# mklarqvist/StormBitmaps

Hardware: AMD Instinct MI355X
Metric: 64-bit bitmap words/s, XX^T upper-tri pairwise AND+popcount (10000x65536) (higher is better)
Workload: dtype u64 (bits as exact FP4 0/1 MFMA operands, f32 accumulate < 2^24); 1 GPU; STORM_contiguous_t N=10000 M=65536 dense draws=32768 seed=42 (BASELINE configs[1], README `benchmark 65536 10000`); entry_point=storm_hip_pairw_dense_launch == STORM_contig_pairw_intersect_cardinality_blocked, kernel_variant=4, work_items=14520

## Files before the change

### stormbitmaps_amd/csrc/storm_hip.hip

```cpp
#include "storm_hip_internal.h"

#include <chrono>

#include <algorithm>
#include <atomic>
#include <cstdarg>
#include <cstdlib>
#include <cstring>

namespace storm {

static thread_local char g_error[512] = "";

void set_error(const char* fmt, ...) {
    va_list ap;
    va_start(ap, fmt);
    vsnprintf(g_error, sizeof(g_error), fmt, ap);
    va_end(ap);
}

#define STORM_PAIR(A, B)                 \
    "v_and_b32 %[t], %[" A "], %[" B "]\n\t" \
    "s_nop 0\n\t"                        \
    "v_bcnt_u32_b32 %[acc], %[t], %[acc]\n\t"
// ... 384 lines not shown
}

int storm_hip_device_pci_bus_id(int device, char* buf, size_t buflen) {
    if (!buf || buflen < 13) return STORM_HIP_EINVAL;
    STORM_HIP_TRY(hipDeviceGetPCIBusId(buf, (int)buflen, device));
    return STORM_HIP_OK;
}

namespace storm {
__global__ void warm_core_kernel() {}
}

int storm_hip_ctx_create(int device, void* stream, storm_hip_ctx_t** out) {
    if (!out) {
        set_error("storm_hip_ctx_create: NULL out");
        return STORM_HIP_EINVAL;
    }
    *out = nullptr;
    int n = 0;
    if (hipGetDeviceCount(&n) != hipSuccess || n == 0) {
        set_error("no HIP device visible (this library has no CPU fallback)");
        return STORM_HIP_ENODEV;
    }
    if (device < 0 || device >= n) {
        set_error("device %d out of range (%d visible)", device, n);
        return STORM_HIP_EINVAL;
    }
    hipDeviceProp_t prop;
    STORM_HIP_TRY(hipGetDeviceProperties(&prop, device));
    if (strncmp(prop.gcnArchName, "gfx950", 6) != 0) {
        set_error("device %d is %s; this library carries gfx950 code objects only", device,
                  prop.gcnArchName);
        return STORM_HIP_ENODEV;
    }
    STORM_HIP_TRY(hipSetDevice(device));
    storm_hip_ctx_t* ctx = new (std::nothrow) storm_hip_ctx_t();
    if (!ctx) return STORM_HIP_ENOMEM;
    ctx->device = device;
    ctx->stream = reinterpret_cast<hipStream_t>(stream);
    ctx->n_cus = prop.multiProcessorCount;
    if (hipMalloc(reinterpret_cast<void**>(&ctx->d_slots), (kSlots + kSlotsExtra) * sizeof(uint64_t)) !=
            hipSuccess ||
        hipMalloc(reinterpret_cast<void**>(&ctx->d_scalar), 64) != hipSuccess) {
        set_error("workspace allocation failed");
        storm_hip_ctx_destroy(ctx);
        return STORM_HIP_ENOMEM;
    }
    if (hipMemsetAsync(ctx->d_slots, 0, (kSlots + kSlotsExtra) * sizeof(uint64_t), ctx->stream) != hipSuccess ||
        hipMemsetAsync(ctx->d_scalar, 0, 64, ctx->stream) != hipSuccess) {
        set_error("workspace memset failed");
        storm_hip_ctx_destroy(ctx);
        return STORM_HIP_EHIP;
    }
    if (!getenv("STORM_HIP_NO_WARM")) {
        hipLaunchKernelGGL(warm_core_kernel, dim3(1), dim3(64), 0, ctx->stream);
        warm_mfma_code(ctx->stream);
        warm_sparse_code(ctx->stream);
        warm_lists_code(ctx->stream);
        (void)result_target(ctx);
        ctx->mail_armed = false;
        (void)hipStreamCreateWithFlags(&ctx->copy_stream, hipStreamNonBlocking);
        {
            std::vector<uint64_t> pageable(kSlots, 0);
            (void)hipMemcpyAsync(ctx->d_slots, pageable.data(), pageable.size() * sizeof(uint64_t), hipMemcpyHostToDevice, ctx->stream);
        }
        if (hipStreamSynchronize(ctx->stream) != hipSuccess || hipGetLastError() != hipSuccess) {
            set_error("warm-up launches failed");
            storm_hip_ctx_destroy(ctx);
            return STORM_HIP_EHIP;
        }
    }
    if (const char* v = getenv("STORM_HIP_VARIANT")) ctx->variant = atoi(v);
    if (const char* v = getenv("STORM_HIP_SEG_ROWS")) ctx->seg_rows = atoi(v);
    if (const char* v = getenv("STORM_HIP_CHUNKS_PER_ITEM")) ctx->chunks_per_item = atoi(v);
    *out = ctx;
    return STORM_HIP_OK;
}

int storm_hip_ctx_set_stream(storm_hip_ctx_t* ctx, void* stream) {
    if (check_ctx(ctx)) return STORM_HIP_EINVAL;
    hipStream_t next = reinterpret_cast<hipStream_t>(stream);
    if (next == ctx->stream) return STORM_HIP_OK;
    STORM_HIP_TRY(hipSetDevice(ctx->device));
    bool ordered = false;
    if (ctx->switch_ev || hipEventCreateWithFlags(&ctx->switch_ev, hipEventDisableTiming) == hipSuccess)
        ordered = hipEventRecord(ctx->switch_ev, ctx->stream) == hipSuccess &&
                  hipStreamWaitEvent(next, ctx->switch_ev, 0) == hipSuccess;
    if (!ordered) {
        (void)hipGetLastError();
        STORM_HIP_TRY(hipStreamSynchronize(ctx->stream));
    }
    ctx->stream = next;
    return STORM_HIP_OK;
}

int storm_hip_ctx_synchronize(storm_hip_ctx_t* ctx) {
    if (check_ctx(ctx)) return STORM_HIP_EINVAL;
    STORM_HIP_TRY(hipSetDevice(ctx->device));
    STORM_HIP_TRY(hipStreamSynchronize(ctx->stream));
    return STORM_HIP_OK;
}

int storm_hip_ctx_reserve_staging(storm_hip_ctx_t* ctx) {
    if (check_ctx(ctx)) return STORM_HIP_EINVAL;
    if (ctx->h_stage_ring) return STORM_HIP_OK;
    STORM_HIP_TRY(hipSetDevice(ctx->device));
    if (hipHostMalloc(&ctx->h_stage_ring, (size_t)24 << 20, hipHostMallocDefault) != hipSuccess) {
        ctx->h_stage_ring = nullptr;
        set_error("reserve_staging: hipHostMalloc of the 24 MiB staging ring failed");
        return STORM_HIP_ENOMEM;
    }
    return STORM_HIP_OK;
}

void storm_hip_ctx_destroy(storm_hip_ctx_t* ctx) {
    if (!ctx) return;
    (void)hipSetDevice(ctx->device);
    drain_deferred(ctx, false);
    if (ctx->d_slots) (void)hipFree(ctx->d_slots);
    if (ctx->d_scalar) (void)hipFree(ctx->d_scalar);
    ctx->d_positions.release();
    if (ctx->h_scalar) (void)hipHostFree(ctx->h_scalar);
    if (ctx->h_mail) (void)hipHostFree(ctx->h_mail);
    if (ctx->h_stage_ring) (void)hipHostFree(ctx->h_stage_ring);
    for (hipEvent_t e : ctx->stage_ev)
        if (e) (void)hipEventDestroy(e);
    if (ctx->switch_ev) (void)hipEventDestroy(ctx->switch_ev);
    ctx->segs.release();
    release_mfma_state(ctx);
    for (hipEvent_t ev : ctx->kernel_events) (void)hipEventDestroy(ev);
    delete ctx;
}

#ifdef STORM_HIP_PROBES
constexpr bool kToolsBuild = true;
#else
constexpr bool kToolsBuild = false;
#endif

struct OptionRow {
    const char* name;
    int storm_hip_ctx_s::*member;
    enum Kind { RANGE, SET, BOOL, ANY, HOOK } kind;
    int64_t lo, hi;
    int64_t step;
    std::vector<int64_t> set;
    const char* text;
    std::vector<int64_t> tools_only;
    const char* tools_text;
    int (*hook)(storm_hip_ctx_t* ctx, int64_t value);
    void (*after)(storm_hip_ctx_t* ctx, int64_t value);
};

static void drop_shadow(storm_hip_ctx_t* ctx, int64_t) { memset(ctx->x4_key, 0, sizeof(ctx->x4_key)); }
static void restart_series(storm_hip_ctx_t* ctx, int64_t value) {
    if (value == 1) ctx->kernel_events_used = 0;
}
static int set_matrix_pad(storm_hip_ctx_t* ctx, int64_t value) {
    ctx->k2_matrix_pad = value < 0 ? -1 : (int)std::min<int64_t>(value, 64);
    return STORM_HIP_OK;
}
static int set_fold_inline(storm_hip_ctx_t* ctx, int64_t value) {
    ctx->k2_fold_inline = value < 0 ? -1 : value != 0;
    return STORM_HIP_OK;
}
static int set_ring(storm_hip_ctx_t* ctx, int64_t value) {
    if (kToolsBuild ? (value < 3 || value > 5) && (value < 11 || value > 18) && value != 26 : value != 4) {
        set_error(kToolsBuild ? "k2_ring must be 3, 4 or 5 (10 + bits = timing probes)"
                              : "k2_ring: this build ships the 4-deep ring only (other depths and the timing "
                                "probes: build with STORM_HIP_PROBES, `make probes`)");
        return STORM_HIP_EINVAL;
    }
    ctx->k2_ring = (int)value;
    return STORM_HIP_OK;
}
static int set_debug(storm_hip_ctx_t* ctx, int64_t value) {
    if (kToolsBuild) {
        ctx->k2_debug = (int)value;
    } else if (value != 0) {
        set_error("k2_debug: timing probes (wrong results by design) are not in this build "
                  "(STORM_HIP_PROBES, `make probes`)");
        return STORM_HIP_EINVAL;
    }
    return STORM_HIP_OK;
}

static const std::vector<OptionRow>& option_table() {
    using C = storm_hip_ctx_s;
    constexpr auto RANGE = OptionRow::RANGE, SET = OptionRow::SET, BOOL = OptionRow::BOOL, ANY = OptionRow::ANY, HOOK = OptionRow::HOOK;
    constexpr const char* kCostText = "%s is a percentage of a full tile's time, 5..100";
    static const std::vector<OptionRow> rows = {
        {"variant", &C::variant, RANGE, -1, 5, 0, {}, "variant must be -1 (auto) or 0..5", {5},
         "variant 5 (wide 32x32x64 strips) is a form of the tools build (`make probes`), not of the shipped library"},
        {"probe_bundle", &C::probe_bundle, SET, 0, 0, 0, {-1, 1, 4},
         "probe_bundle must be -1 (auto: 1), 1 (one group of 128 rows per workgroup) or 4 (bundles of four)"},
        {"sparse_probe", &C::sparse_probe, RANGE, -1, 1, 0, {}, "sparse_probe must be -1 (auto), 0 (never) or 1 (every eligible column)"},
        {"result_mailbox", &C::result_mailbox, BOOL},
        {"sync_poll_us", &C::sync_poll_us, RANGE, 0, 1000000, 0, {}, "sync_poll_us: 0 .. 1000000 microseconds"},
        {"matrix_lists", &C::matrix_lists, RANGE, -1, 1, 0, {}, "matrix_lists must be -1 (by density), 0 (never) or 1 (whenever eligible)"},
        {"matrix_lists_kernel", &C::matrix_lists_kernel, RANGE, 0, 2, 0, {},
         "matrix_lists_kernel: 0 (by the row length), 1 (window kernel) or 2 (hash kernel)"},
        {"matrix_lists_hash_min_log2", &C::matrix_lists_hash_min_log2, RANGE, 3, 7, 0, {}, "matrix_lists_hash_min_log2: 3 .. 7"},
        {"matrix_lists_debug", &C::matrix_lists_debug, ANY},
        {"matrix_lists_density", &C::matrix_lists_permille_x10, RANGE, 0, 10000, 0, {},
         "matrix_lists_density: 0 .. 10000 (1/10000 of the dense replica's bits)"},
        {"seg_rows", &C::seg_rows, RANGE, 1, 1 << 20, 0, {}, "seg_rows out of range"},
        {"k2_stages_per_item", &C::k2_stages_per_item, RANGE, 1, 65536, 0, {}, "k2_stages_per_item out of range"},
        {"k2_max_run", &C::k2_max_run, RANGE, 0, 4096, 0, {},
         "k2_max_run out of range (0 = chosen by the list-scheduling estimate, 1..4096)"},
        {"k2_ring", &C::k2_ring, HOOK, 0, 0, 0, {}, nullptr, {}, nullptr, set_ring},
        {"k2_shadow_budget_mb", &C::k2_shadow_budget_mb, RANGE, 0, 1 << 22, 0, {}, "k2_shadow_budget_mb must be 0 (unbounded) .. 4194304",
         {}, nullptr, nullptr, drop_shadow},
        {"k2_tile_shape", &C::k2_tile_shape, SET, 0, 0, 0, {0, 1, 2, 3, 4, 5, 6, 16, 32},
         "k2_tile_shape must be 0 (chosen by the matrix), 5 (both operands as FP4 images in the LDS, 16x16x128 MFMAs), 1, 2 (bit operands inflated in registers), 3 / 4 (B as FP4 images in the LDS, 16x16x128 / 32x32x64 MFMAs), 6 (128 x 128 tiles, k-parts whose sums meet inside the launch), 16 or 32 (FP4 shadow)",
         {1, 16},
         "k2_tile_shape = 1 / 16 (tilebits_kernel, tile16_fp4_kernel) is a form of the tools build (`make probes`), not of the shipped library"},
        {"k2_ring_sync", &C::k2_ring_sync, BOOL},
        {"k2_wave_below", &C::k2_wave_below, RANGE, 0, 1 << 30, 0, {}, "k2_wave_below: 0 (never) .. 2^30 tiles of 256 x 256"},
        {"k2_part_slots", &C::k2_part_slots, RANGE, 0, 2, 0, {}, "k2_part_slots must be 0 (by the length of the segments), 1 or 2 per CU"},
        {"k2_part_min_chunks", &C::k2_part_min_chunks, RANGE, 1, 4096, 0, {}, "k2_part_min_chunks: 1 .. 4096 chunks of 512 bits"},
        {"k2_part_narrow", &C::k2_part_narrow, BOOL},
        {"k2_part_cost_diag", &C::k2_part_cost_diag, RANGE, 10, 100, 0, {}, "k2_part_cost_diag: 10 .. 100 percent of a full tile's chunk"},
        {"k2_ring_cost_diag", &C::k2_ring_cost_diag, RANGE, 5, 100, 0, {}, kCostText},
        {"k2_ring_cost_ragged", &C::k2_ring_cost_ragged, RANGE, 5, 100, 0, {}, kCostText},
        {"k2_tile_cost_diag", &C::k2_tile_cost_diag, RANGE, 5, 100, 0, {}, kCostText},
        {"k2_tile_cost_ragged", &C::k2_tile_cost_ragged, RANGE, 5, 100, 0, {}, kCostText},
        {"k2_strip_operands", &C::k2_strip_operands, RANGE, 0, 6, 0, {},
         "k2_strip_operands must be 0 (by size), 1 (bit operands, one item per workgroup), 2 (bit operands, one stream per workgroup), 3 (the same with a ring per wave), 4 (FP4 shadow), 5 (bit operands, FP4 image built in the LDS) or 6 (the same with 512-row A tiles, two halves behind one image)",
         {1, 3},
         "k2_strip_operands = 1 (stripbits_kernel) and 3 (bitwave_kernel) are forms of the tools build (`make probes`), not of the shipped library"},
        {"k2_strip_rows", &C::k2_strip_rows, SET, 0, 0, 0, {0, 64, 128},
         "k2_strip_rows must be 0 (by rule), 64 (64 A rows per wave, 256-row A tiles) or 128 (128 A rows per wave on 128-bit slices, 512-row A tiles)"},
        {"k2_shard_pairs", &C::k2_shard_pairs, BOOL},
        {"k2_matrix_pad", &C::k2_matrix_pad, HOOK, 0, 0, 0, {}, nullptr, {}, nullptr, set_matrix_pad},
        {"k2_fold_inline", &C::k2_fold_inline, HOOK, 0, 0, 0, {}, nullptr, {}, nullptr, set_fold_inline},
        {"k2_wave_ring", &C::k2_wave_ring, SET, 0, 0, 0, {0, 3, 4, 6, 8}, "k2_wave_ring must be 0 (by occupancy), 3, 4, 6 or 8"},
        {"k2_stream_max_rows", &C::k2_stream_max_rows, RANGE, 0, 1ll << 31, 0, {}, "k2_stream_max_rows must be 0 .. 2^31"},
        {"k2_stream_groups_per_cu", &C::k2_stream_groups_per_cu, RANGE, 0, 255, 0, {}, "k2_stream_groups_per_cu must be 0 (auto) .. 255"},
        {"k2_stream_min_piece", &C::k2_stream_min_piece, RANGE, 1, 4096, 0, {}, "%s must be 1..4096 stages"},
        {"k2_stream_min_run", &C::k2_stream_min_run, RANGE, 1, 4096, 0, {}, "%s must be 1..4096 stages"},
        {"k2_stream_w3_1", &C::k2_stream_w3_1, RANGE, 10, 1000, 0, {}, "%s must be 10..1000 percent of the first workgroup's share"},
        {"k2_stream_w3_2", &C::k2_stream_w3_2, RANGE, 10, 1000, 0, {}, "%s must be 10..1000 percent of the first workgroup's share"},
        {"k2_shape", &C::k2_shape, SET, 0, 0, 0, {16, 32}, "k2_shape must be 16 (16x16x128 MFMA) or 32 (32x32x64)", {32},
         "k2_shape = 32 (strip_fp4_kernel) is a form of the tools build (`make probes`), not of the shipped library"},
        {"keep_shadow", &C::keep_shadow, BOOL, 0, 0, 0, {}, nullptr, {}, nullptr, nullptr, drop_shadow},
        {"k2_matrix_parts", &C::k2_matrix_parts, BOOL},
        {"k2_matrix_min_part", &C::k2_matrix_min_part, RANGE, 4, 4096, 4, {},
         "k2_matrix_min_part: a multiple of 4 in 4 .. 4096 (stages of 128 bits)"},
        {"k2_matrix_split", &C::k2_matrix_split, BOOL},
        {"k2_pitch_pad", &C::k2_pitch_pad, RANGE, -1, 65536, 128, {}, "k2_pitch_pad must be -1 (auto) or a multiple of 128 in 0..65536"},
        {"k2_lds_pad", &C::k2_lds_pad, RANGE, 0, 120 * 1024, 0, {}, "k2_lds_pad must be 0..122880"},
        {"k2_persistent", &C::k2_persistent, BOOL, 0, 0, 0, {}, nullptr, {1},
         "k2_persistent (strip_fp4_kernel with work queues) is a form of the tools build (`make probes`), not of the shipped library"},
        {"k2_lpt_rounds", &C::k2_lpt_rounds, RANGE, 0, 63, 0, {}, "k2_lpt_rounds must be 0..63"},
        {"k2_tail_slices", &C::k2_tail_slices, RANGE, 0, 255, 0, {}, "k2_tail_slices must be 0..255"},
        {"k2_tail_run", &C::k2_tail_run, RANGE, 1, 4096, 0, {}, "k2_tail_run must be 1..4096"},
        {"k2_debug", &C::k2_debug, HOOK, 0, 0, 0, {}, nullptr, {}, nullptr, set_debug},
        {"time_kernels", &C::time_kernels, BOOL, 0, 0, 0, {}, nullptr, {}, nullptr, nullptr, restart_series},
        {"chunks_per_item", &C::chunks_per_item, RANGE, 0, 4096, 0, {}, "chunks_per_item out of range"},
    };
    return rows;
}

static const OptionRow* find_option(const char* key) {
    for (const OptionRow& row : option_table())
        if (!strcmp(key, row.name)) return &row;
    return nullptr;
}

int storm_hip_option_check(const char* key, int64_t value) {
    storm_hip_ctx_s scratch;
    scratch.n_cus = 256;
    return storm_hip_ctx_set_option(&scratch, key, value);
}

int storm_hip_ctx_set_option(storm_hip_ctx_t* ctx, const char* key, int64_t value) {
    if (check_ctx(ctx) || !key) return STORM_HIP_EINVAL;
    const OptionRow* row = find_option(key);
    if (!row) {
        set_error("unknown option '%s'", key);
        return STORM_HIP_EINVAL;
    }
    if (row->kind == OptionRow::HOOK) return row->hook(ctx, value);
    const auto among = [](const std::vector<int64_t>& set, int64_t v) { return std::find(set.begin(), set.end(), v) != set.end(); };
    const int64_t stored = row->kind == OptionRow::BOOL ? value != 0 : value;
    if ((row->kind == OptionRow::RANGE && (value < row->lo || value > row->hi || (row->step && value > 0 && value % row->step))) ||
        (row->kind == OptionRow::SET && !among(row->set, value))) {
        set_error(row->text, key);
        return STORM_HIP_EINVAL;
    }
    if (!kToolsBuild && among(row->tools_only, stored)) {
        set_error(row->tools_text, key);
        return STORM_HIP_EINVAL;
    }
    ctx->*(row->member) = (int)stored;
    if (row->after) row->after(ctx, value);
    return STORM_HIP_OK;
}

int64_t storm_hip_ctx_get_option(storm_hip_ctx_t* ctx, const char* key) {
    if (check_ctx(ctx) || !key) return -1;
    if (const OptionRow* row = find_option(key)) return ctx->*(row->member);
    if (!strcmp(key, "variant_used")) return ctx->variant_used;
    if (!strcmp(key, "k2_operands_used")) return ctx->k2_operands_used;
    if (!strcmp(key, "k2_strip_rows_used")) return ctx->k2_strip_rows_used;
    if (!strcmp(key, "k2_tile_shape_used")) return ctx->k2_tile_shape_eff;
    if (!strcmp(key, "n_cus")) return ctx->n_cus;
    if (!strcmp(key, "probes_build") || !strcmp(key, "probes_built")) return kToolsBuild;
    return -1;
}

int storm_hip_kernel_time(storm_hip_ctx_t* ctx, double* sum_ms, uint64_t* launches) {
    if (check_ctx(ctx) || !sum_ms || !launches) return STORM_HIP_EINVAL;
    STORM_HIP_TRY(hipSetDevice(ctx->device));
    STORM_HIP_TRY(hipStreamSynchronize(ctx->stream));
    *sum_ms = 0.0;
    *launches = 0;
    for (size_t i = 0; i + 1 < ctx->kernel_events_used; i += 2) {
        float ms = 0.f;
        STORM_HIP_TRY(hipEventElapsedTime(&ms, ctx->kernel_events[i], ctx->kernel_events[i + 1]));
        *sum_ms += ms;
        ++*launches;
    }
    ctx->kernel_events_used = 0;
    return STORM_HIP_OK;
}

int storm_hip_debug_strip_trace(storm_hip_ctx_t* ctx, uint64_t* out, uint64_t capacity_items,
                                uint64_t* n_items) {
    return guarded("storm_hip_debug_strip_trace", [&]() -> int {
    if (check_ctx(ctx) || !n_items) return STORM_HIP_EINVAL;
#ifndef STORM_HIP_PROBES
    set_error("strip trace: not in this build (STORM_HIP_PROBES, `make probes`)");
    *n_items = 0;
    return STORM_HIP_EINVAL;
#endif
    *n_items = ctx->trace_items;
    if (!out || ctx->trace_items == 0) return STORM_HIP_OK;
    STORM_HIP_TRY(hipSetDevice(ctx->device));
    STORM_HIP_TRY(hipStreamSynchronize(ctx->stream));
    const uint64_t n = std::min<uint64_t>(capacity_items, ctx->trace_items);
    if (ctx->trace_is_stream) {
        STORM_HIP_TRY(hipMemcpy(out, ctx->d_trace, n * 8 * sizeof(uint64_t), hipMemcpyDeviceToHost));
        return STORM_HIP_OK;
    }
    std::vector<uint64_t> raw(n * 4);
    std::vector<uint32_t> items(n * 5, 0);
    STORM_HIP_TRY(hipMemcpy(raw.data(), ctx->d_trace, n * 4 * sizeof(uint64_t), hipMemcpyDeviceToHost));
    if (!ctx->trace_is_stream)
        STORM_HIP_TRY(hipMemcpy(items.data(), ctx->strips.d, n * 5 * sizeof(uint32_t),
                                hipMemcpyDeviceToHost));
    for (uint64_t i = 0; i < n; ++i) {
        for (int k = 0; k < 4; ++k) out[i * 8 + k] = raw[i * 4 + k];
        out[i * 8 + 4] = items[i * 5 + 0];
        out[i * 8 + 5] = items[i * 5 + 1];
        out[i * 8 + 6] = (uint64_t)items[i * 5 + 3] - items[i * 5 + 2];
        out[i * 8 + 7] = items[i * 5 + 4];
    }
    return STORM_HIP_OK;
    });
}

int storm_hip_last_pass_report(storm_hip_ctx_t* ctx, uint64_t out[4]) {
    if (check_ctx(ctx) || !out) return STORM_HIP_EINVAL;
    memcpy(out, ctx->pass_report, sizeof(ctx->pass_report));
    return STORM_HIP_OK;
}

int storm_hip_last_launch_info(storm_hip_ctx_t* ctx, uint64_t out[4]) {
    if (check_ctx(ctx) || !out) return STORM_HIP_EINVAL;
    memcpy(out, ctx->last_info, sizeof(ctx->last_info));
    return STORM_HIP_OK;
}

int storm_hip_matrix_create(storm_hip_ctx_t* ctx, uint64_t n_rows, uint32_t n_words,
                            storm_hip_matrix_t** out) {
    return guarded("storm_hip_matrix_create", [&]() -> int {
    if (check_ctx(ctx) || !out) return STORM_HIP_EINVAL;
    *out = nullptr;
    if (n_words == 0 || n_rows >= (1ull << 32) - kABlockRows) {
        set_error("matrix shape out of range (rows=%llu words=%u)", (unsigned long long)n_rows,
                  n_words);
        return STORM_HIP_EINVAL;
    }
    STORM_HIP_TRY(hipSetDevice(ctx->device));
    storm_hip_matrix_t* m = new (std::nothrow) storm_hip_matrix_t();
    if (!m) return STORM_HIP_ENOMEM;
    m->n_rows = n_rows;
    m->n_words = n_words;
    m->generation = next_matrix_generation();
    m->n_rows_pad = std::max<uint64_t>(kRowPad, (n_rows + kRowPad - 1) / kRowPad * kRowPad);
    m->stride_words = ((uint64_t)n_words + kChunkWords - 1) / kChunkWords * kChunkWords;
    m->stride_words += pitch_pad_chunks(ctx->k2_matrix_pad, m->stride_words) * kChunkWords;
    const size_t bytes = m->n_rows_pad * m->stride_words * sizeof(uint64_t);
    if (hipMalloc(reinterpret_cast<void**>(&m->d), bytes) != hipSuccess) {
        set_error("hipMalloc of %zu bytes for the dense matrix failed", bytes);
        delete m;
        return STORM_HIP_ENOMEM;
    }
    if (hipMemsetAsync(m->d, 0, bytes, ctx->stream) != hipSuccess) {
        set_error("hipMemsetAsync failed");
        (void)hipFree(m->d);
        delete m;
        return STORM_HIP_EHIP;
    }
    *out = m;
    return STORM_HIP_OK;
    });
}

int storm_hip_matrix_resize(storm_hip_ctx_t* ctx, storm_hip_matrix_t* m, uint64_t n_rows) {
    return guarded("storm_hip_matrix_resize", [&]() -> int {
    if (check_ctx(ctx)) return STORM_HIP_EINVAL;
    if (!m || n_rows >= (1ull << 32) - kABlockRows) {
        set_error("matrix_resize: NULL matrix or row count out of range");
        return STORM_HIP_EINVAL;
    }
    STORM_HIP_TRY(hipSetDevice(ctx->device));
    const uint64_t row_bytes = m->stride_words * sizeof(uint64_t);
    if (n_rows > m->n_rows_pad) {
        const uint64_t want = (n_rows + kRowPad - 1) / kRowPad * kRowPad;
        const uint64_t new_pad = std::max<uint64_t>(want, 2 * m->n_rows_pad);
        uint64_t* nd = nullptr;
        if (hipMalloc(reinterpret_cast<void**>(&nd), new_pad * row_bytes) != hipSuccess) {
            set_error("matrix_resize: hipMalloc of %llu bytes failed",
                      (unsigned long long)(new_pad * row_bytes));
            return STORM_HIP_ENOMEM;
        }
        if (hipMemcpyAsync(nd, m->d, m->n_rows_pad * row_bytes, hipMemcpyDeviceToDevice,
                           ctx->stream) != hipSuccess ||
            hipMemsetAsync(nd + m->n_rows_pad * m->stride_words, 0,
                           (new_pad - m->n_rows_pad) * row_bytes, ctx->stream) != hipSuccess ||
            hipStreamSynchronize(ctx->stream) != hipSuccess) {
            (void)hipFree(nd);
            set_error("matrix_resize: device copy failed");
            return STORM_HIP_EHIP;
        }
        (void)hipFree(m->d);
        m->d = nd;
        m->n_rows_pad = new_pad;
    } else if (n_rows < m->n_rows) {
        STORM_HIP_TRY(hipMemsetAsync(m->d + n_rows * m->stride_words, 0,
                                     (m->n_rows - n_rows) * row_bytes, ctx->stream));
    }
    m->n_rows = n_rows;
    m->generation = next_matrix_generation();
    return STORM_HIP_OK;
    });
}

static int check_rows(const storm_hip_matrix_t* m, uint64_t row0, uint64_t n_rows) {
    if (!m) {
        set_error("NULL matrix");
        return STORM_HIP_EINVAL;
    }
    if (row0 + n_rows > m->n_rows || row0 + n_rows < row0) {
        set_error("rows [%llu, +%llu) outside the matrix (%llu rows)", (unsigned long long)row0,
                  (unsigned long long)n_rows, (unsigned long long)m->n_rows);
        return STORM_HIP_EINVAL;
// ... 684 lines not shown
```

### stormbitmaps_amd/csrc/storm_hip_internal.h

```cpp
#pragma once

#include <hip/hip_runtime.h>

#include <algorithm>
#include <cstdint>
#include <cstdio>
#include <exception>
#include <cstring>
#include <new>
#include <optional>
#include <thread>
#include <utility>
#include <variant>
#include <vector>

#include "storm_hip.h"
#include "storm_hip_plan.h"

struct storm_hip_ctx_s;
typedef struct storm_hip_ctx_s storm_hip_ctx_t;
struct storm_hip_matrix_s;

namespace storm {

// ... 49 lines not shown
            return STORM_HIP_ENOMEM;
        }
        capacity = bytes;
        return STORM_HIP_OK;
    }
    void release() {
        if (d) (void)hipFree(d);
        d = nullptr;
        capacity = 0;
    }
};

template <class Rec, class Key>
struct WorkList {
    DevBuf<Rec> d;
    std::optional<Key> key;
    uint32_t n = 0;
    const Rec* recs() const { return d.d; }
    bool holds(const Key& k) const { return d && key == k; }
    void forget() {
        key.reset();
        n = 0;
    }
    template <class R>
    int put(storm_hip_ctx_t* ctx, std::optional<Key>&& k, const R* recs, size_t count, const char* what, size_t floor_bytes = 0);
    void release() {
        d.release();
        forget();
    }
};

struct SegRequest {
    uint64_t n_rows;
    uint32_t shard_rank, shard_count, seg_len;
    bool operator==(const SegRequest& o) const {
        return n_rows == o.n_rows && shard_rank == o.shard_rank && shard_count == o.shard_count && seg_len == o.seg_len;
    }
};
struct SegList : WorkList<Seg, SegRequest> {
    uint64_t row_sum = 0;
};

struct ItemList : WorkList<void, std::variant<TileSumRequest, MatrixTilesRequest, Tile128Request>> {
    MatrixPlan matrix_plan;
    template <class Rq>
    bool holds(const Rq& rq) const {
        const Rq* have = key ? std::get_if<Rq>(&*key) : nullptr;
        return d && have && *have == rq;
    }
};

struct StripList : WorkList<StripItem, StripRequest> {
    uint32_t queue_base[8] = {0, 0, 0, 0, 0, 0, 0, 0};
    uint32_t queue_count[8] = {0, 0, 0, 0, 0, 0, 0, 0};
};

struct PanelList {
    WorkList<StripItem, StripRequest> list;
    hipEvent_t landed = nullptr;
};

constexpr int kLanes = 64;
constexpr int kWaves = 4;
constexpr int kThreads = kLanes * kWaves;
constexpr int kRowsPerWave = 32;
static_assert(kABlockRows == kWaves * kRowsPerWave, "128 A rows per workgroup (storm_hip_plan.h)");
constexpr int kRowPad = 256;
constexpr int kStageRows = 32;
constexpr int kSlots = 4096;
constexpr int kSlotsExtra = 8;

int launch_pairw_segments(storm_hip_ctx_t* ctx, const uint64_t* X, uint64_t stride_words,
                          const Seg* d_segs, uint32_t n_segs, uint64_t seg_row_sum,
                          uint64_t* d_total);

}

struct storm_hip_ctx_s {
    int device = 0;
    hipStream_t stream = nullptr;
    hipEvent_t switch_ev = nullptr;
    int n_cus = 0;
    unsigned long long* d_slots = nullptr;
    unsigned long long* d_scalar = nullptr;
    unsigned long long* h_scalar = nullptr;
    unsigned long long* h_mail = nullptr;
    unsigned long long* d_mail = nullptr;
    int result_mailbox = 1;
    int sync_poll_us = 0;
    bool mail_armed = false;
    std::vector<void*> deferred_free, deferred_host_free;
    uint32_t deferred_age = 0;
    hipEvent_t stage_ev[3] = {nullptr, nullptr, nullptr};
    bool stage_used[3] = {false, false, false};
    int stage_next = 0;
    void* h_stage_ring = nullptr;
    storm::SegList segs;
    int variant = -1;
    int variant_used = 2;
    int probe_bundle = -1;
    int sparse_probe = -1;
    int matrix_lists = -1;
    int matrix_lists_kernel = 0;
    int matrix_lists_hash_min_log2 = 6;
    int matrix_lists_debug = 0;
    int matrix_lists_permille_x10 = 80;
    int seg_rows = 256;
    int chunks_per_item = 0;
    uint64_t last_info[4] = {0, 0, 0, 0};
    uint64_t sparse_census[4] = {0, 0, 0, 0};
    uint64_t pass_report[4] = {0, 0, 0, 0};
    storm::DevBuf<uint8_t> d_x4;
    storm::ItemList items;
    std::vector<storm::PanelList> panel_lists;
    hipStream_t copy_stream = nullptr;
    storm::StripList strips;
    int k2_stages_per_item = 32;
    int k2_max_run = 0;
    int k2_ring = 4;
    int k2_shadow_budget_mb = 96 * 1024;
    int k2_strip_operands = 0;
    int k2_stream_max_rows = 8192;
    int k2_shard_pairs = 0;
    int k2_matrix_pad = -1;
    int k2_fold_inline = -1;
    int k2_operands_used = 4;
    int k2_strip_rows = 0;
    int k2_strip_rows_used = 64;
    int k2_tile_shape = 0;
    int k2_wave_below = 400;
    int k2_part_slots = 0;
    int k2_part_min_chunks = 8;
    int k2_part_narrow = 1;
    int k2_part_cost_diag = 80;
    storm::DevBuf<uint32_t> d_tickets;
    bool tickets_dirty = false;
    int k2_tile_shape_eff = 2;
    int k2_ring_sync = 0;
    int k2_ring_cost_diag = 78, k2_ring_cost_ragged = 40;
    int k2_tile_cost_diag = 63, k2_tile_cost_ragged = 30;
    int k2_shape = 16;
    int k2_persistent = 0;
    int keep_shadow = 0;
    uint64_t x4_key[4] = {0, 0, 0, 0};
    int k2_matrix_split = 1;
    int k2_matrix_parts = 0;
    storm::DevBuf<uint32_t> d_parts;
    int k2_matrix_min_part = 32;
    int k2_pitch_pad = -1;
    int k2_lds_pad = 0;
    int k2_lpt_rounds = 6;
    int k2_tail_slices = 3;
    int k2_tail_run = 32;
    int time_kernels = 0;
    std::vector<hipEvent_t> kernel_events;
    size_t kernel_events_used = 0;
    storm::DevBuf<uint32_t> d_band;
    storm::DevBuf<uint64_t> d_dosage_rows;
    storm::DevBuf<uint32_t> d_dosage_sums;
    storm::DevBuf<void> d_positions;
    storm::DevBuf<uint32_t> d_counts;
    storm::DevBuf<unsigned long long> d_trace;
    uint32_t trace_items = 0;
    storm::WorkList<uint32_t, storm::BitstreamRequest> bitfirst;
    storm::DevBuf<storm::BitSeg> d_bitsegs;
    uint32_t n_bit_groups = 0, n_bit_segs = 0, bit_max_stages = 0;
    uint64_t bit_stages = 0;
    int k2_stream_groups_per_cu = 0;
    int k2_stream_min_piece = 6;
    int k2_stream_min_run = 2;
    int k2_stream_w3_1 = 120, k2_stream_w3_2 = 60;
    int k2_wave_ring = 0;
    bool trace_is_stream = false;
    int k2_debug = 0;
};

namespace storm {
int launch_pairw_mfma(storm_hip_ctx_t* ctx, const storm_hip_matrix_s* m, uint32_t shard_rank,
                      uint32_t shard_count, uint64_t* d_total);
int launch_pairw_mfma_ranges(storm_hip_ctx_t* ctx, const uint64_t* X, uint64_t stride_words,
                             uint64_t n_rows_src, uint64_t n_rows_dst,
                             const std::vector<RowRange>& ranges, uint32_t shard_rank,
                             uint32_t shard_count, int strip_mode, uint64_t* d_total,
                             uint64_t shadow_generation = 0, uint32_t n_words_logical = 0);
int launch_pairw_bits_upload(storm_hip_ctx_t* ctx, storm_hip_matrix_s* m, const uint64_t* host_rows,
                             uint64_t src_stride_words, uint64_t* d_total);
int stage_check_lists(const storm_hip_stage_s* stage, const std::vector<uint64_t>& ltable);
int stage_gather_lists(storm_hip_ctx_t* ctx, storm_hip_stage_s* stage, const std::vector<uint64_t>& ltable, uint16_t* d_lists,
                       uint64_t** d_table);
int strip_operands_of(const storm_hip_ctx_t* ctx);
int launch_pairw_bits_ranges(storm_hip_ctx_t* ctx, const uint8_t* X, uint64_t pitch_bytes,
                             const std::vector<RowRange>& ranges, uint32_t n_kslices2, uint32_t shard_rank,
                             uint32_t shard_count, uint64_t* d_total, bool slots_hold_sums = false,
                             uint32_t a_tile = 256u,
                             bool rows128 = false);
static inline uint64_t ranges_word_pairs(const std::vector<RowRange>& ranges, uint64_t words, uint32_t shard_count) {
    uint64_t pairs = 0;
    for (const RowRange& rg : ranges) {
        const uint64_t n = rg.r1 - rg.r0, a = rg.a_end ? std::min(rg.a_end, rg.r1) - rg.r0 : n;
        pairs += a * (a - (a != 0)) / 2 + a * (n - a);
    }
    return pairs * words / (shard_count ? shard_count : 1);
}
int launch_pairw_matrix(storm_hip_ctx_t* ctx, const storm_hip_matrix_s* m, int op, uint32_t* d_out,
                        uint64_t ld, uint64_t band_row0 = 0, uint64_t band_rows = ~0ull);
int launch_pairw_lag_matrix(storm_hip_ctx_t* ctx, const storm_hip_matrix_s* m, int op, uint64_t max_lag, uint64_t band_row0,
                            uint64_t band_rows, uint32_t* d_out, uint64_t ld);
int launch_pairw_dosage_matrix(storm_hip_ctx_t* ctx, const storm_hip_matrix_s* m, uint32_t* d_out, uint64_t ld);
int launch_pairw_lag_dosage_matrix(storm_hip_ctx_t* ctx, const storm_hip_matrix_s* m, uint64_t max_lag, uint64_t band_row0,
                                   uint64_t band_rows, uint32_t* d_out, uint64_t ld);
int launch_square_dosage_matrix(storm_hip_ctx_t* ctx, const storm_hip_matrix_s* a, const storm_hip_matrix_s* b, uint32_t* d_out,
                                uint64_t ld);
int launch_square_mfma(storm_hip_ctx_t* ctx, const storm_hip_matrix_s* a,
                       const storm_hip_matrix_s* b, uint64_t* d_total);
int launch_square_matrix(storm_hip_ctx_t* ctx, const storm_hip_matrix_s* a,
                         const storm_hip_matrix_s* b, int op, uint32_t* d_out, uint64_t ld);
int launch_row_counts(storm_hip_ctx_t* ctx, const storm_hip_matrix_s* m, uint32_t* d_counts);
int launch_similarity_finish(storm_hip_ctx_t* ctx, void* d_io, uint64_t ld, uint64_t n_rows, uint64_t n_cols,
                             const uint32_t* d_counts_rows, const uint32_t* d_counts_cols, int triangle, int measure,
                             uint64_t n_bits);
int launch_similarity_finish_lag(storm_hip_ctx_t* ctx, void* d_io, uint64_t ld, uint64_t n_rows, uint64_t row0,
                                 uint64_t n_band_rows, uint64_t max_lag, const uint32_t* d_counts, int measure, uint64_t n_bits);
int launch_lag_band_sums(storm_hip_ctx_t* ctx, const float* d_vals, uint64_t ld, uint64_t n_rows, uint64_t max_lag, int stat,
                         uint64_t n_const, const uint32_t* d_nobs, uint64_t nobs_row_pitch, uint64_t nobs_col_stride,
                         float* d_score, uint32_t* d_n_pairs);
constexpr uint32_t kLdscoreMaxAnnot = 1024;
int launch_lag_band_annot_sums(storm_hip_ctx_t* ctx, const float* d_vals, uint64_t ld, uint64_t n_rows, uint64_t max_lag, int stat,
                               uint64_t n_const, const uint32_t* d_nobs, uint64_t nobs_row_pitch, uint64_t nobs_col_stride,
                               const uint32_t* d_lo, const uint32_t* d_hi, const float* d_annot, uint64_t annot_ld,
                               uint64_t n_annot, float* d_score, uint64_t score_ld, uint32_t* d_n_pairs);
int check_lag_band_prune(const char* who, uint64_t n_rows, const uint32_t* h_lo, const uint32_t* h_hi, float min_r2);
size_t lag_band_prune_scratch_words(uint64_t n_rows, uint64_t lag, bool windows, bool order);
int launch_lag_band_prune(storm_hip_ctx_t* ctx, const char* who, const float* d_vals, uint64_t ld, uint64_t n_rows, uint64_t lag,
                          float min_r2, const uint32_t* h_lo, const uint32_t* h_hi, const uint32_t* h_order, uint8_t* d_keep,
                          uint32_t* d_owner, uint32_t* d_scratch);
void release_mfma_state(storm_hip_ctx_t* ctx);
void drain_deferred(storm_hip_ctx_t* ctx, bool aged);
void warm_mfma_code(hipStream_t stream);
void warm_sparse_code(hipStream_t stream);
void warm_lists_code(hipStream_t stream);
int fetch_result_word(storm_hip_ctx_t* ctx, uint64_t* h_total);
uint64_t* result_target(storm_hip_ctx_t* ctx);
int wait_mailbox(storm_hip_ctx_t* ctx, uint64_t* value);
int launch_fold_slots(storm_hip_ctx_t* ctx, uint64_t* d_total);
void kernel_time_mark(storm_hip_ctx_t* ctx);
uint64_t next_matrix_generation();
struct Piece { const void* src; size_t bytes; size_t dst_off; size_t zero_after = 0; };
struct Stager {
    static constexpr size_t kBuf = 8u << 20;
    static constexpr int kBufs = 3;
    storm_hip_ctx_t* ctx;
    hipEvent_t (&ev)[kBufs];
    bool (&used)[kBufs];
    int& next;
    explicit Stager(storm_hip_ctx_t* c) : ctx(c), ev(c->stage_ev), used(c->stage_used), next(c->stage_next) {}
    static_assert(kBuf * kBufs == ((size_t)24 << 20), "storm_hip_ctx_reserve_staging allocates the same ring");
    int init() {
        if (!ctx->h_stage_ring) {
            if (hipHostMalloc(&ctx->h_stage_ring, kBuf * kBufs, hipHostMallocDefault) != hipSuccess) {
                ctx->h_stage_ring = nullptr;
                set_error("sparse_create: hipHostMalloc of the %zu-byte staging ring failed", kBuf * kBufs);
                return STORM_HIP_ENOMEM;
            }
        }
        for (int i = 0; i < kBufs; ++i)
            if (!ev[i] && hipEventCreateWithFlags(&ev[i], hipEventDisableTiming) != hipSuccess) return STORM_HIP_EHIP;
        return STORM_HIP_OK;
    }
    int send(uint8_t* d_base, const Piece* pieces, size_t n, size_t span) {
        uint8_t* buf = static_cast<uint8_t*>(ctx->h_stage_ring) + (size_t)next * kBuf;
        if (used[next] && hipEventSynchronize(ev[next]) != hipSuccess) return STORM_HIP_EHIP;
        const unsigned parts = span >= (1u << 20) ? 4u : 1u;
        auto pack = [&](unsigned part) {
            for (size_t i = n * part / parts; i < n * (part + 1) / parts; ++i) {
                memcpy(buf + pieces[i].dst_off, pieces[i].src, pieces[i].bytes);
                if (pieces[i].zero_after) memset(buf + pieces[i].dst_off + pieces[i].bytes, 0, pieces[i].zero_after);
            }
        };
        if (parts > 1) {
            std::thread helpers[3];
            for (unsigned t = 1; t < parts; ++t) helpers[t - 1] = std::thread(pack, t);
            pack(0);
            for (unsigned t = 1; t < parts; ++t) helpers[t - 1].join();
        } else {
            pack(0);
        }
        if (hipMemcpyAsync(d_base, buf, span, hipMemcpyHostToDevice, ctx->stream) != hipSuccess ||
            hipEventRecord(ev[next], ctx->stream) != hipSuccess)
            return STORM_HIP_EHIP;
        used[next] = true;
        next = (next + 1) % kBufs;
        return STORM_HIP_OK;
    }
    int send_rows(uint8_t* d_base, const std::vector<const void*>& rows, size_t bytes, size_t stride) {
        const size_t per_chunk = kBuf / stride;
        std::vector<Piece> chunk;
        for (size_t r0 = 0; r0 < rows.size(); r0 += per_chunk) {
            const size_t n = std::min(per_chunk, rows.size() - r0);
            chunk.clear();
            for (size_t i = 0; i < n; ++i) chunk.push_back({rows[r0 + i], bytes, i * stride, stride - bytes});
            if (int rc = send(d_base + r0 * stride, chunk.data(), n, n * stride)) return rc;
        }
        return STORM_HIP_OK;
    }
    int send_run(uint8_t* d_base, const std::vector<std::pair<const void*, size_t>>& run) {
        std::vector<Piece> chunk;
// ... 115 lines not shown
```

### stormbitmaps_amd/csrc/storm_hip_mfma.hip

```cpp
#include "storm_hip_internal.h"

#include <algorithm>
#include <chrono>
#include <cstring>
#include <exception>
#include <type_traits>
#include <utility>

namespace storm {

#ifdef STORM_HIP_PROBES
__device__ unsigned long long g_clock_probe[4];
#define STORM_CLOCK_BEGIN()                                  \
    const uint64_t ck_t0 = __builtin_amdgcn_s_memtime();     \
    const uint64_t ck_r0 = __builtin_amdgcn_s_memrealtime()
#define STORM_CLOCK_END()                                                                           \
    do {                                                                                            \
        if (threadIdx.x == 0) {                                                                     \
            atomicAdd(&g_clock_probe[0], (unsigned long long)(__builtin_amdgcn_s_memtime() - ck_t0)); \
            atomicAdd(&g_clock_probe[1], (unsigned long long)(__builtin_amdgcn_s_memrealtime() - ck_r0)); \
            atomicAdd(&g_clock_probe[2], 1ull);                                                     \
        }                                                                                           \
    } while (0)
#else
// ... 1010 lines not shown
            STORM_BS_FETCH(x1, t, 1, 0);
            STORM_BS_FETCH(x2, t, 0, 1);
            STORM_BS_FETCH(x3, t, 1, 1);
            asm volatile("s_waitcnt lgkmcnt(0)" : "+v"(x1), "+v"(x2), "+v"(x3)::"memory");
            __builtin_amdgcn_sched_barrier(0);
            a[0][0][0] = tb_inflate<0>(w0); a[0][1][0] = tb_inflate<1>(w0);
            a[0][2][0] = tb_inflate<2>(w0); a[0][3][0] = tb_inflate<3>(w0);
            a[0][0][1] = tb_inflate<0>(x1); a[0][1][1] = tb_inflate<1>(x1);
            a[0][2][1] = tb_inflate<2>(x1); a[0][3][1] = tb_inflate<3>(x1);
            a[1][0][0] = tb_inflate<0>(x2); a[1][1][0] = tb_inflate<1>(x2);
            a[1][2][0] = tb_inflate<2>(x2); a[1][3][0] = tb_inflate<3>(x2);
            a[1][0][1] = tb_inflate<0>(x3); a[1][1][1] = tb_inflate<1>(x3);
            a[1][2][1] = tb_inflate<2>(x3); a[1][3][1] = tb_inflate<3>(x3);
            if (diag) {
#pragma unroll
                for (int k = 0; k < 4; ++k)
                    dbits += __builtin_popcount((uint32_t)w0[k]) + __builtin_popcount((uint32_t)x1[k]) +
                             __builtin_popcount((uint32_t)x2[k]) + __builtin_popcount((uint32_t)x3[k]);
            }
        }
        if (mul) {
            const int half = (own && ci < 4u) ? 1 : 0;
            sb[0] = tb_scale<0>() - half;
            sb[1] = tb_scale<1>() - half;
            sb[2] = tb_scale<2>() - half;
            sb[3] = tb_scale<3>() - half;
            __builtin_amdgcn_sched_barrier(0);
            STORM_BS_STAGE(t, tn);
            STORM_BS_WAIT();
            STORM_BS_KEEP();
        } else {
            STORM_BS_FETCH(w0, tn, 0, 0);
            asm volatile("s_waitcnt lgkmcnt(0)" : "+v"(w0)::"memory");
            __builtin_amdgcn_sched_barrier(0);
            e0 = tb_inflate<0>(w0);
        }
        if (kTrace) {
            const unsigned long long now = __builtin_readcyclecounter();
            c_body += now - c_mark;
            c_mark = now;
            n_mul += mul ? 1u : 0u;
        }
        if (kTrace) c_issue += __builtin_readcyclecounter() - c_mark;
        ++t;
        ++ci;
        if (ci == 4u + rc.n_b) {
            ci = 0;
            ++sc;
            rc = segs[min(sc, s_end - 1u)];
        }
    }
#undef STORM_BS_STAGE
#undef STORM_BS_KEEP
#undef STORM_BS_WAIT
#undef STORM_BS_STEP
#undef STORM_BS_FETCH

    long long mine2 = 0;
#pragma unroll
    for (int m = 0; m < 2; ++m) {
        uint32_t part = 0;
#pragma unroll
        for (int n = 0; n < 2; ++n)
#pragma unroll
            for (int r = 0; r < 16; ++r) part += (uint32_t)(acc[m][n][r] * 2.0f);
        mine2 += part;
    }
    mine2 -= (long long)dbits;
#pragma unroll
    for (int o = 32; o > 0; o >>= 1) mine2 += __shfl_down(mine2, o, 64);
    __builtin_amdgcn_s_barrier();
    long long* wsum = reinterpret_cast<long long*>(lds_raw);
    if (lane == 0) wsum[wave] = mine2;
    __syncthreads();
    if (tid == 0) {
        const long long tot2 = wsum[0] + wsum[1] + wsum[2] + wsum[3];
        if (tot2 != 0) atomicAdd(&slots[blockIdx.x & (kBsFoldSlots - 1)], (unsigned long long)(tot2 / 2));
        __threadfence();
        const unsigned long long arrived = atomicAdd(&slots[kBsTicket], 1ull);
        wsum[4] = (arrived == (unsigned long long)gridDim.x - 1ull) ? 1 : 0;
        if (kTrace) {
            trace[blockIdx.x * 8ull + 0] = t_start;
            trace[blockIdx.x * 8ull + 1] = __builtin_amdgcn_s_memrealtime();
            trace[blockIdx.x * 8ull + 2] = ((t_ready - t_start) & 0xffffffffull) | ((unsigned long long)t << 32);
            trace[blockIdx.x * 8ull + 3] = __builtin_amdgcn_s_getreg(20 | (0 << 6) | (31 << 11)) |
                                           ((unsigned long long)__builtin_amdgcn_s_getreg(4 | (0 << 6) | (31 << 11)) << 32);
            trace[blockIdx.x * 8ull + 4] = c_wait;
            trace[blockIdx.x * 8ull + 5] = c_issue;
            trace[blockIdx.x * 8ull + 6] = c_body;
            trace[blockIdx.x * 8ull + 7] = n_mul;
        }
    }
    __syncthreads();
    if (wsum[4] != 0 && wave == 0) {
        __threadfence();
        unsigned long long v = __hip_atomic_exchange(&slots[lane], 0ull, __ATOMIC_RELAXED, __HIP_MEMORY_SCOPE_AGENT);
#pragma unroll
        for (int o = 32; o > 0; o >>= 1) v += __shfl_down(v, o, 64);
        if (lane == 0) {
            out[0] = v;
            __hip_atomic_store(&slots[kBsTicket], 0ull, __ATOMIC_RELAXED, __HIP_MEMORY_SCOPE_AGENT);
        }
    }
}

#ifdef STORM_HIP_PROBES
#include "../../tools/probes/bitwave.hip"
#endif

static void release_panel_lists(storm_hip_ctx_t* ctx) {
    for (PanelList& l : ctx->panel_lists) {
        l.list.release();
        if (l.landed) (void)hipEventDestroy(l.landed);
    }
    ctx->panel_lists.clear();
    if (ctx->copy_stream) (void)hipStreamDestroy(ctx->copy_stream);
    ctx->copy_stream = nullptr;
}

__global__ void warm_mfma_kernel() {}
void warm_mfma_code(hipStream_t stream) { hipLaunchKernelGGL(warm_mfma_kernel, dim3(1), dim3(64), 0, stream); }

void release_mfma_state(storm_hip_ctx_t* ctx) {
    release_panel_lists(ctx);
    ctx->d_x4.release();
    ctx->items.release();
    ctx->strips.release();
    ctx->d_trace.release();
    ctx->d_counts.release();
    ctx->d_band.release();
    ctx->d_dosage_rows.release();
    ctx->d_dosage_sums.release();
    ctx->d_parts.release();
    ctx->d_tickets.release();
    ctx->d_bitsegs.release();
    ctx->bitfirst.release();
}

constexpr size_t kItemsFloorBytes = 4096 * sizeof(MfmaItem);
constexpr size_t kStripItemsFloorBytes = 4096 * sizeof(StripItem);

static int ensure_items(storm_hip_ctx_t* ctx, const std::vector<RowRange>& ranges,
                        uint32_t total_stages, uint32_t shard_rank, uint32_t shard_count,
                        bool diag_only) {
    const TileSumRequest rq = {ranges_hash(ranges), total_stages, shard_rank, shard_count,
                               (uint32_t)std::max(1, ctx->k2_stages_per_item), diag_only ? 1u : 0u,
                               (ctx->k2_debug & 3) == 1 ? 1u : 0u};
    if (ctx->items.holds(rq)) return STORM_HIP_OK;
    std::vector<MfmaItem> items;
    if (int rc = plan_tile_sum(rq, ranges, items)) return rc;
    return ctx->items.put(ctx, rq, items.data(), items.size(), "K2: the item table", kItemsFloorBytes);
}

static StripOptions strip_options_of(const storm_hip_ctx_t* ctx, int xcd_group) {
    StripOptions o;
    o.max_run = ctx->k2_max_run;
    o.tail_run = ctx->k2_tail_run;
    o.tail_slices = ctx->k2_tail_slices;
    o.lpt_rounds = ctx->k2_lpt_rounds;
    o.shard_pairs = ctx->k2_shard_pairs != 0;
    o.n_cus = ctx->n_cus;
    o.xcd_group = xcd_group;
    o.persistent = ctx->k2_persistent != 0;
    o.one_slice_probe = (ctx->k2_debug & 16) != 0;
    return o;
}

static int ensure_strip_items(storm_hip_ctx_t* ctx, const std::vector<RowRange>& ranges,
                              uint32_t n_kslices, uint32_t shard_rank, uint32_t shard_count,
                              uint32_t a_tile, int xcd_group = 1) {
    const StripRequest rq = strip_request(strip_options_of(ctx, xcd_group), ranges, n_kslices, shard_rank, shard_count, a_tile);
    if (ctx->strips.holds(rq)) return STORM_HIP_OK;
    ctx->strips.forget();
    std::vector<StripItem> items;
    plan_strips(rq, ranges, items, ctx->strips.queue_base, ctx->strips.queue_count);
    if (items.size() >= (1ull << 31)) {
        set_error("K2s: %zu strip items exceed the grid limit", items.size());
        return STORM_HIP_EINVAL;
    }
    return ctx->strips.put(ctx, rq, items.data(), items.size(), "K2s: the strip items", kStripItemsFloorBytes);
}

static uint64_t shadow_pitch(const storm_hip_ctx_t* ctx, uint64_t row_bytes) {
    if (ctx->k2_pitch_pad >= 0) return row_bytes + (uint64_t)ctx->k2_pitch_pad;
    return row_bytes + (row_bytes % 1024 == 0 ? 384u : 0u);
}
static int ensure_shadow(storm_hip_ctx_t* ctx, size_t bytes, const char* what) {
    if (bytes > ctx->d_x4.capacity) memset(ctx->x4_key, 0, sizeof(ctx->x4_key));
    return ctx->d_x4.ensure(bytes, what);
}

int launch_pairw_mfma_ranges(storm_hip_ctx_t* ctx, const uint64_t* X, uint64_t stride_words,
                             uint64_t n_rows_src, uint64_t n_rows_dst,
                             const std::vector<RowRange>& ranges, uint32_t shard_rank,
                             uint32_t shard_count, int strip_mode, uint64_t* d_total,
                             uint64_t shadow_generation, uint32_t n_words_logical) {
    const bool strips = strip_mode != 0;
    const uint32_t a_tile = strip_mode == 2 ? 512u : (uint32_t)kStripATile;
    const uint64_t row_bytes = stride_words * 32;
    const uint32_t n_kslices = n_words_logical
                                   ? (n_words_logical + 3u) / 4u
                                   : (uint32_t)(row_bytes / kStripRowBytes);
    const uint64_t rows_alloc = std::max<uint64_t>(n_rows_dst, kTile);
    uint32_t n_chunks = 1, chunk_slices = n_kslices;
    uint64_t shadow_row_bytes = row_bytes;
    if (strips) {
        uint64_t want = 1;
        if (ctx->k2_shadow_budget_mb > 0) {
            const uint64_t budget = (uint64_t)ctx->k2_shadow_budget_mb << 20;
            const uint64_t full = rows_alloc * shadow_pitch(ctx, row_bytes);
            if (full > budget && n_kslices > 8) want = (full + budget - 1) / budget;
        }
        constexpr uint32_t kDmaCapSlices = ((1u << 26) - 1024u) / kStripRowBytes / 8u * 8u;
        want = std::max<uint64_t>(want, ((uint64_t)n_kslices + kDmaCapSlices - 1) / kDmaCapSlices);
        if (want > 1) {
            chunk_slices = (uint32_t)(((uint64_t)n_kslices + want - 1) / want + 7u) / 8u * 8u;
            chunk_slices = std::min(chunk_slices, kDmaCapSlices);
            n_chunks = (n_kslices + chunk_slices - 1) / chunk_slices;
            shadow_row_bytes = (uint64_t)chunk_slices * kStripRowBytes;
        }
    }
    const uint64_t pitch = shadow_pitch(ctx, shadow_row_bytes);
    const size_t x4_bytes = (size_t)rows_alloc * pitch;
    if (n_rows_dst / kTile >= 65535) {
        set_error("K2: too many row blocks");
        return STORM_HIP_EINVAL;
    }
    if (int rc = ensure_shadow(ctx, x4_bytes, "K2: the FP4 shadow matrix")) return rc;
    const uint32_t total_stages = (uint32_t)(row_bytes / kStageBytes);
    if (strips) {
        ctx->items.forget();
    } else if (int rc = ensure_items(ctx, ranges, total_stages, shard_rank, shard_count, false)) {
        return rc;
    }
    if (pitch * (uint64_t)(strips ? kStripBRows : kTile) >= (1ull << 32)) {
        set_error("K2: rows of %llu nibble bytes exceed the 32-bit DMA offsets; use variant 2",
                  (unsigned long long)shadow_row_bytes);
        return STORM_HIP_EINVAL;
    }
    if (strips)
        if (int rc = ensure_strip_items(ctx, ranges, chunk_slices, shard_rank, shard_count, a_tile))
            return rc;
    if ((uint64_t)ctx->k2_stages_per_item * 128u >= (1u << 24)) {
        set_error("K2: k-slice too long for exact f32 accumulation");
        return STORM_HIP_EINVAL;
    }
    const uint32_t n_strip = strips ? ctx->strips.n : 0;
    const uint32_t n_tiles = ctx->items.n;
    const uint64_t key[4] = {(uint64_t)(uintptr_t)X, shadow_generation,
                             ((uint64_t)shard_rank << 32) | shard_count,
                             (pitch << 20) ^ (n_rows_dst << 2) ^ (uint64_t)strip_mode};
    const bool shadow_valid = ctx->keep_shadow && shadow_generation != 0 && n_chunks == 1 &&
                              !memcmp(key, ctx->x4_key, sizeof(key)) &&
                              (ctx->k2_debug >> 8) == 0;
    const ExpandOwn own = strips ? ExpandOwn{shard_rank, shard_count, 5u,
                                             ctx->k2_shard_pairs ? 0u
                                                                 : strip_modulo_slices(chunk_slices, shard_count) / kOwnSlices}
                                 : ExpandOwn{shard_rank, shard_count, 7u, 0xffffffffu};
    const uint32_t nib = (ctx->k2_debug >> 8) ? (uint32_t)(ctx->k2_debug >> 8) & 15u : 2u;
    const uint64_t n_src = std::min(n_rows_src, n_rows_dst);
    for (uint32_t chunk = 0; chunk < n_chunks && (n_tiles > 0 || n_strip > 0); ++chunk) {
        if (!shadow_valid) {
            if (n_chunks == 1) {
                hipLaunchKernelGGL(expand_fp4_kernel,
                                   expand_grid(n_rows_dst, stride_words, expand_compact_halves(own, stride_words * 2)),
                                   dim3(256), 0, ctx->stream, X, stride_words, n_src, n_rows_dst,
                                   reinterpret_cast<uint4*>(ctx->d_x4.d), own, nib, pitch / 16);
            } else {
                const uint64_t h0 = (uint64_t)chunk * chunk_slices * 8u, h1 = h0 + (uint64_t)chunk_slices * 8u;
                hipLaunchKernelGGL(expand_fp4_kernel,
                                   expand_grid(n_rows_dst, stride_words, expand_compact_halves(own, h1 - h0)),
                                   dim3(256), 0, ctx->stream, X, stride_words, n_src, n_rows_dst,
                                   reinterpret_cast<uint4*>(ctx->d_x4.d), own, nib, pitch / 16, h0, h1, h0);
            }
        }
        STORM_HIP_TRY(hipGetLastError());
        if (n_chunks == 1) memcpy(ctx->x4_key, key, sizeof(key));
        else memset(ctx->x4_key, 0, sizeof(ctx->x4_key));
        if (n_strip > 0) {
            kernel_time_mark(ctx);
            const StripItem* sit = ctx->strips.d;
            const dim3 sgrid(n_strip), sblock(kStripThreads);
#ifdef STORM_HIP_PROBES
            StripQueues queues;
            memcpy(queues.base, ctx->strips.queue_base, sizeof(queues.base));
            memcpy(queues.count, ctx->strips.queue_count, sizeof(queues.count));
            unsigned int* heads = reinterpret_cast<unsigned int*>(ctx->d_slots + kSlots);
            const dim3 pgrid(std::min<uint32_t>(n_strip, (uint32_t)ctx->n_cus * (strip_mode == 2 ? 2u : 4u)));
            const bool persist = ctx->k2_persistent && n_chunks == 1;
            const int sel = strip_mode == 2 ? 100 + ctx->k2_ring
                                            : (persist && ctx->k2_ring == 4) ? 204
                                            : (persist && ctx->k2_ring == 18) ? 218
                                                                              : ctx->k2_ring;
            switch (sel) {
#include "../../tools/probes/strip_fp4_32_launch.hip"
                default:
                    if (ctx->k2_shape != 16)
                        hipLaunchKernelGGL(strip_fp4_kernel<kStripRingDefault>, sgrid, sblock,
                                           (size_t)ctx->k2_lds_pad, ctx->stream, ctx->d_x4, pitch, sit,
                                           ctx->d_slots);
                    else
                        hipLaunchKernelGGL(strip16_fp4_kernel<kStripRingDefault>, sgrid, sblock,
                                           (size_t)ctx->k2_lds_pad, ctx->stream, ctx->d_x4, pitch, sit,
                                           ctx->d_slots);
                    break;
            }
#else
            hipLaunchKernelGGL(strip16_fp4_kernel<kStripRingDefault>, sgrid, sblock, (size_t)ctx->k2_lds_pad, ctx->stream,
                               ctx->d_x4, pitch, sit, ctx->d_slots);
#endif
            kernel_time_mark(ctx);
            STORM_HIP_TRY(hipGetLastError());
        }
        if (n_tiles > 0) {
            kernel_time_mark(ctx);
            const dim3 kgrid(n_tiles), block(kMfmaThreads);
            const MfmaItem* items = static_cast<const MfmaItem*>(ctx->items.recs());
            switch (ctx->k2_debug & 12) {
#ifdef STORM_HIP_PROBES
                case 4:
                    hipLaunchKernelGGL(pairw_fp4_kernel<4>, kgrid, block, 0, ctx->stream, ctx->d_x4,
                                       pitch, items, ctx->d_slots);
                    break;
                case 8:
                    hipLaunchKernelGGL(pairw_fp4_kernel<8>, kgrid, block, 0, ctx->stream, ctx->d_x4,
                                       pitch, items, ctx->d_slots);
                    break;
#endif
// ... 392 lines not shown
int launch_square_matrix(storm_hip_ctx_t* ctx, const storm_hip_matrix_s* a,
                         const storm_hip_matrix_s* b, int op, uint32_t* d_out, uint64_t ld) {
    if (a->n_rows == 0 || b->n_rows == 0) return STORM_HIP_OK;
    ctx->k2_tile_shape_eff = (ctx->k2_tile_shape && ctx->k2_tile_shape != 6) ? ctx->k2_tile_shape : ((a->sparse_origin && b->sparse_origin) ? 2 : 5);
    const uint64_t stride_words = a->stride_words;
    const uint64_t row_bytes = stride_words * 32;
    const bool bits = ctx->k2_tile_shape_eff <= 5 && b->stride_words == stride_words;
    const uint64_t pitch = bits ? stride_words * 8 : shadow_pitch(ctx, row_bytes);
    const uint64_t rows_a = (a->n_rows + kTile - 1) / kTile * kTile;
    const uint64_t rows_b = (b->n_rows + kTile - 1) / kTile * kTile;
    if (int rc = check_tile_limits("square_matrix", pitch, kTile, (rows_a + rows_b) / kTile + 1, false)) return rc;
    const size_t x4_bytes = bits ? 0 : (size_t)(rows_a + rows_b) * pitch;
    if (int rc = ensure_shadow(ctx, x4_bytes, "square_matrix: the FP4 shadow")) return rc;
    const uint32_t total_stages = bits ? (std::max(a->n_words, b->n_words) + 7u) / 8u * 4u : (uint32_t)(row_bytes / kStageBytes);
    const uint32_t ta = (uint32_t)(rows_a / kTile), tb = (uint32_t)(rows_b / kTile);
    const bool k2h = choose_tile128(ctx, (uint64_t)ta * tb, pitch, bits);
    int rc = STORM_HIP_OK;
    MatrixPlan plan;
    if (k2h) {
        ctx->k2_tile_shape_eff = 6;
    } else {
        MatrixTilesRequest rq;
        rq.total_stages = total_stages;
        xcd_grouped_tiles(0, ta, ta, ta + tb, false, rq.tiles);
        rc = ensure_matrix_tiles(ctx, std::move(rq), &plan);
    }
    uint32_t* d_counts = nullptr;
    if (rc == STORM_HIP_OK) rc = op_row_counts(ctx, op, a, b, rows_a, rows_a + rows_b, &d_counts);
    if (rc == STORM_HIP_OK) {
        const OutWindow w = rectangle_window(d_out, ld, a->n_rows, rows_a, b->n_rows, d_counts, op);
        for (int side = 0; side < 2 && !bits; ++side) {
            const storm_hip_matrix_s* m = side ? b : a;
            const uint64_t rows_dst = side ? rows_b : rows_a;
            const dim3 grid = expand_grid(rows_dst, stride_words);
            hipLaunchKernelGGL(expand_fp4_kernel, grid, dim3(256), 0, ctx->stream, m->d,
                               stride_words, std::min<uint64_t>(m->n_rows_pad, rows_dst), rows_dst,
                               reinterpret_cast<uint4*>(ctx->d_x4.d + (side ? rows_a * pitch : 0)),
                               kExpandAll, 2u, pitch / 16);
        }
        const TileOperands ops = bits ? operands_of(a->d, b->d, pitch, rows_a, std::min<uint64_t>(a->n_rows_pad, rows_a),
                                                    std::min<uint64_t>(b->n_rows_pad, rows_b))
                                      : operands_of(ctx->d_x4.d, pitch, rows_a + rows_b);
        rc = k2h ? run_tile128(ctx, total_stages, ops, w, 1u) : run_matrix_tiles(ctx, plan, ops, bits, w);
    }
    if (rc == STORM_HIP_EHIP) set_error("square_matrix: HIP failure");
    return rc;
}

static BitstreamRequest bitstream_request_of(const storm_hip_ctx_t* ctx, const std::vector<RowRange>& ranges, uint32_t n_kslices,
                                             uint32_t shard_rank, uint32_t shard_count, uint64_t pitch) {
    BitstreamShaping sh;
    sh.groups_per_cu = ctx->k2_stream_groups_per_cu;
    sh.min_piece = std::max(1, ctx->k2_stream_min_piece);
    sh.min_run = std::max(1, ctx->k2_stream_min_run);
    sh.w3_1 = ctx->k2_stream_w3_1;
    sh.w3_2 = ctx->k2_stream_w3_2;
    return bitstream_request(sh, ranges, n_kslices, shard_rank, shard_count, (uint32_t)std::max(1, ctx->n_cus), pitch);
}

static int ensure_bitstream(storm_hip_ctx_t* ctx, const std::vector<RowRange>& ranges, uint32_t n_kslices,
                            uint32_t shard_rank, uint32_t shard_count, uint64_t pitch) {
    const BitstreamRequest rq = bitstream_request_of(ctx, ranges, n_kslices, shard_rank, shard_count, pitch);
    if (ctx->bitfirst.holds(rq)) return STORM_HIP_OK;
    ctx->bitfirst.forget();
    BitstreamPlan plan;
    build_bitstream(rq, ranges, plan);
    if (plan.bases.size() >= (1ull << 32) ||
        (!ranges.empty() && ranges.back().r1 * pitch / 64 + n_kslices >= (1ull << 32))) {
        set_error("K2q: the matrix is beyond the 32-bit stage addresses (64-byte units)");
        return STORM_HIP_EINVAL;
    }
    if (plan.max_stages > kBsMaxStages) {
        set_error("K2q: a workgroup of %u stages exceeds the exact range of its accumulators", plan.max_stages);
        return STORM_HIP_EINVAL;
    }
    const size_t seg_bytes = std::max<size_t>(plan.segs.size(), 1) * sizeof(BitSeg);
    std::vector<uint32_t> packed(plan.first);
    packed.insert(packed.end(), plan.first_stage.begin(), plan.first_stage.end());
    packed.insert(packed.end(), plan.bases.begin(), plan.bases.end());
    packed.push_back(0u);
    if (int rc = ctx->d_bitsegs.ensure(seg_bytes, "K2q: the segment table")) return rc;
    if (upload_bytes(ctx, ctx->d_bitsegs, plan.segs.data(), plan.segs.size() * sizeof(BitSeg))) {
        set_error("K2q: the segment table: the copy to the device failed");
        return STORM_HIP_EHIP;
    }
    ctx->n_bit_groups = plan.groups;
    ctx->bit_stages = plan.stages;
    ctx->bit_max_stages = plan.max_stages;
    ctx->n_bit_segs = (uint32_t)plan.segs.size();
    return ctx->bitfirst.put(ctx, rq, packed.data(), packed.size(), "K2q: the workgroups' stage tables");
}

int launch_pairw_bitstream(storm_hip_ctx_t* ctx, const uint64_t* X, uint64_t pitch,
                           const std::vector<RowRange>& ranges, uint32_t n_kslices, uint32_t shard_rank,
                           uint32_t shard_count, uint64_t* d_total) {
    if (pitch * (uint64_t)kStripBRows >= (1ull << 32) || pitch % 64 != 0) {
        set_error("K2q: rows of %llu bytes are outside the bit-operand stream's 32-bit DMA offsets",
                  (unsigned long long)pitch);
        return STORM_HIP_EINVAL;
    }
    if (int rc = ensure_bitstream(ctx, ranges, n_kslices, shard_rank, shard_count, pitch)) return rc;
    ctx->pass_report[0] |= STORM_HIP_RAN_BITSTREAM;
    ctx->pass_report[1] += ranges_word_pairs(ranges, (uint64_t)n_kslices * 8u, shard_count);
    ctx->items.forget();
    ctx->last_info[0] = ctx->n_bit_groups;
    ctx->last_info[1] = ctx->bit_max_stages;
    ctx->last_info[2] = 1;
    ctx->last_info[3] = ctx->n_bit_segs;
    if (ctx->n_bit_groups == 0)
        return launch_fold_slots(ctx, d_total);
    kernel_time_mark(ctx);
    const dim3 grid(ctx->n_bit_groups), block(kStripThreads);
#ifdef STORM_HIP_PROBES
    if (ctx->k2_ring == 18) {
        const size_t need = (size_t)ctx->n_bit_groups * 8 * sizeof(unsigned long long);
        if (int rc = ctx->d_trace.ensure(need, "K2q: the schedule trace")) return rc;
        ctx->trace_items = ctx->n_bit_groups;
        ctx->trace_is_stream = true;
        hipLaunchKernelGGL(bitstream_kernel<true>, grid, block, 0, ctx->stream,
                           reinterpret_cast<const uint8_t*>(X), pitch, ctx->d_bitsegs.d,
                           ctx->bitfirst.recs(),
                           ctx->bitfirst.recs() + 2 * ((size_t)ctx->n_bit_groups + 1),
                           ctx->bitfirst.recs() + ((size_t)ctx->n_bit_groups + 1), ctx->d_slots,
                           reinterpret_cast<unsigned long long*>(d_total), ctx->d_trace);
    } else
#endif
        hipLaunchKernelGGL(bitstream_kernel<false>, grid, block, 0, ctx->stream,
                           reinterpret_cast<const uint8_t*>(X), pitch, ctx->d_bitsegs.d,
                           ctx->bitfirst.recs(),
                           ctx->bitfirst.recs() + 2 * ((size_t)ctx->n_bit_groups + 1),
                           ctx->bitfirst.recs() + ((size_t)ctx->n_bit_groups + 1), ctx->d_slots,
                           reinterpret_cast<unsigned long long*>(d_total), (unsigned long long*)nullptr);
    kernel_time_mark(ctx);
    STORM_HIP_TRY(hipGetLastError());
    return STORM_HIP_OK;
}

#ifdef STORM_HIP_PROBES
#include "../../tools/probes/bitwave_launch.hip"
#endif

int launch_pairw_bits_ranges(storm_hip_ctx_t* ctx, const uint8_t* X, uint64_t pitch,
                             const std::vector<RowRange>& ranges, uint32_t n_kslices2, uint32_t shard_rank,
                             uint32_t shard_count, uint64_t* d_total, bool slots_hold_sums, uint32_t a_tile, bool rows128) {
    if (pitch * (uint64_t)kStripBRows >= (1ull << 32)) {
        set_error("K2b: rows of %llu bytes are beyond the strips' 32-bit DMA offsets", (unsigned long long)pitch);
        return STORM_HIP_EINVAL;
    }
    ctx->items.forget();
    if (rows128 && a_tile != kStripRowsATile) {
        set_error("K2b: the 128-rows-per-wave form takes A tiles of 512 rows");
        return STORM_HIP_EINVAL;
    }
    if (int rc = ensure_strip_items(ctx, ranges, n_kslices2, shard_rank, shard_count, a_tile, rows128 ? (int)kStripRowsXcdGroup : 2))
        return rc;
    const uint32_t n_strip = ctx->strips.n;
    const uint32_t waves = rows128 ? 4u : a_tile / (uint32_t)kStripBRows;
    ctx->k2_operands_used = waves == 8u ? 6 : 5;
    ctx->k2_strip_rows_used = rows128 ? 128 : 64;
    if (n_strip > 0) {
        ctx->pass_report[0] |= STORM_HIP_RAN_BIT_STRIPS;
        ctx->pass_report[1] += ranges_word_pairs(ranges, (uint64_t)n_kslices2 * (rows128 ? 2u : 4u), shard_count);
    }
    ctx->last_info[0] = n_strip;
    ctx->last_info[1] = ctx->k2_stages_per_item;
    ctx->last_info[2] = 1;
    ctx->last_info[3] = 0;
    const uint32_t fold_slots = n_strip <= 4096u ? 256u : (uint32_t)kSlots;
    const bool fold_wanted = ctx->k2_fold_inline > 0 || (ctx->k2_fold_inline < 0 && n_strip <= 4096u);
    const uint64_t arrivals_per_slot = (uint64_t)n_strip * (uint64_t)waves / (uint64_t)fold_slots + 1u;
    const uint64_t wave_sum_max = rows128 ? 128ull * (4096ull * 64ull + 512ull) * 128ull
                                          : 64ull * (4096ull * 64ull + 256ull) * 256ull;
    const bool fold_inline = fold_wanted && !slots_hold_sums && n_strip > 0 && arrivals_per_slot < 65535u &&
                             arrivals_per_slot * wave_sum_max < (1ull << 48);
    if (n_strip > 0) {
        kernel_time_mark(ctx);
        if (rows128) {
            const bool plain = ranges.size() == 1 && ranges[0].r0 == 0 && ranges[0].a_end == 0 && ranges[0].back_from == ~0ull &&
                               ranges[0].r1 < (uint64_t)kStripRowsNoTrim;
            hipLaunchKernelGGL(strip16_rows_kernel, dim3(n_strip), dim3(256), (size_t)ctx->k2_lds_pad,
                               ctx->stream, X, pitch, ctx->strips.recs(), ctx->d_slots,
                               fold_inline ? reinterpret_cast<unsigned long long*>(d_total) : nullptr, fold_slots,
                               plain ? (uint32_t)ranges[0].r1 : kStripRowsNoTrim);
        } else if (waves == 8u)
            hipLaunchKernelGGL(strip16_bits2_kernel, dim3(n_strip), dim3(512), (size_t)ctx->k2_lds_pad,
                               ctx->stream, X, pitch, ctx->strips.recs(), ctx->d_slots,
                               fold_inline ? reinterpret_cast<unsigned long long*>(d_total) : nullptr, fold_slots);
        else
            hipLaunchKernelGGL(strip16_bits_kernel, dim3(n_strip), dim3(kStripThreads), (size_t)ctx->k2_lds_pad,
                               ctx->stream, X, pitch, ctx->strips.recs(), ctx->d_slots,
                               fold_inline ? reinterpret_cast<unsigned long long*>(d_total) : nullptr, fold_slots);
        kernel_time_mark(ctx);
        STORM_HIP_TRY(hipGetLastError());
    }
    return fold_inline ? STORM_HIP_OK : launch_fold_slots(ctx, d_total);
}

static bool strip_rows128_by_rule(const storm_hip_matrix_s* m, uint32_t shard_count) {
    return shard_count == 1 && m->n_rows >= 2048 && m->n_words >= 1024;
}
static bool strip_rows128(const storm_hip_ctx_t* ctx, const storm_hip_matrix_s* m, uint32_t shard_count) {
    if (ctx->k2_strip_rows == 64 || ctx->k2_strip_operands == 6 || (m->n_rows + kStripRowsATile - 1) / kStripRowsATile * kStripRowsATile > m->n_rows_pad) return false;
    return ctx->k2_strip_rows == 128 || strip_rows128_by_rule(m, shard_count);
}

static int launch_pairw_bits(storm_hip_ctx_t* ctx, const storm_hip_matrix_s* m, uint32_t shard_rank,
                             uint32_t shard_count, int operands, uint64_t* d_total) {
    const uint64_t pitch = m->stride_words * 8;
    const uint64_t n_rows4 = (m->n_rows + kStripATile - 1) / kStripATile * kStripATile;
    if (n_rows4 > m->n_rows_pad || pitch * (uint64_t)kStripBRows >= (1ull << 32)) {
        set_error("K2sb: matrix of %llu rows (%llu allocated) x %llu bytes per row is outside the bit-operand strips' reach",
                  (unsigned long long)m->n_rows, (unsigned long long)m->n_rows_pad, (unsigned long long)pitch);
        return STORM_HIP_EINVAL;
    }
    std::vector<RowRange> ranges;
    if (m->n_rows > 1) ranges.push_back({0, m->n_rows});
    const uint32_t n_kslices = (m->n_words + 7u) / 8u;
    if (operands == 2)
        return launch_pairw_bitstream(ctx, m->d, pitch, ranges, n_kslices, shard_rank, shard_count, d_total);
#ifdef STORM_HIP_PROBES
    if (operands == 3)
        return launch_pairw_bitwave(ctx, m->d, pitch, ranges, n_kslices, shard_rank, shard_count, d_total);
#endif
    ctx->items.forget();
    if (operands == 5 && strip_rows128(ctx, m, shard_count))
        return launch_pairw_bits_ranges(ctx, reinterpret_cast<const uint8_t*>(m->d), pitch, ranges, strip_rows_kslices(m->n_words),
                                        shard_rank, shard_count, d_total, false, kStripRowsATile, true);
    if (operands == 5 || operands == 6)
        return launch_pairw_bits_ranges(ctx, reinterpret_cast<const uint8_t*>(m->d), pitch, ranges, n_kslices * 2u,
                                        shard_rank, shard_count, d_total, false, operands == 6 ? 512u : (uint32_t)kStripATile, false);
    if (int rc = ensure_strip_items(ctx, ranges, n_kslices, shard_rank, shard_count, (uint32_t)kStripATile))
        return rc;
#ifndef STORM_HIP_PROBES
    set_error("k2_strip_operands = 1 (stripbits_kernel) is in the tools build only (`make probes`)");
    return STORM_HIP_EINVAL;
#else
    const uint32_t n_strip = ctx->strips.n;
    if (n_strip > 0) {
        kernel_time_mark(ctx);
        hipLaunchKernelGGL(stripbits_kernel, dim3(n_strip), dim3(kStripThreads), 0, ctx->stream,
                           reinterpret_cast<const uint8_t*>(m->d), pitch,
                           ctx->strips.recs(), ctx->d_slots);
        kernel_time_mark(ctx);
        STORM_HIP_TRY(hipGetLastError());
    }
    ctx->last_info[0] = n_strip;
    ctx->last_info[1] = ctx->k2_stages_per_item;
    ctx->last_info[2] = 1;
    ctx->last_info[3] = 0;
    return launch_fold_slots(ctx, d_total);
#endif
}

static int pairw_bits_upload_queue(storm_hip_ctx_t* ctx, storm_hip_matrix_s* m, const uint64_t* host_rows,
                                   uint64_t src_stride_words, uint64_t* d_total);
int launch_pairw_bits_upload(storm_hip_ctx_t* ctx, storm_hip_matrix_s* m, const uint64_t* host_rows,
                             uint64_t src_stride_words, uint64_t* d_total) {
    const int rc = pairw_bits_upload_queue(ctx, m, host_rows, src_stride_words, d_total);
    if (rc != STORM_HIP_OK) {
        if (ctx->copy_stream) (void)hipStreamSynchronize(ctx->copy_stream);
        (void)hipStreamSynchronize(ctx->stream);
        ctx->mail_armed = false;
    }
    return rc;
}
static int pairw_bits_upload_queue(storm_hip_ctx_t* ctx, storm_hip_matrix_s* m, const uint64_t* host_rows,
                                   uint64_t src_stride_words, uint64_t* d_total) {
    const uint64_t pitch = m->stride_words * 8;
    const uint64_t tiles = (m->n_rows + kStripATile - 1) / kStripATile;
    if (tiles * kStripATile > m->n_rows_pad || pitch * (uint64_t)kStripBRows >= (1ull << 32) || m->n_rows < 2) {
        set_error("pairw_dense_upload: matrix outside the bit-operand strips' reach");
        return STORM_HIP_EINVAL;
    }
    if (!ctx->copy_stream) STORM_HIP_TRY(hipStreamCreateWithFlags(&ctx->copy_stream, hipStreamNonBlocking));
    std::vector<PanelList>& lists = ctx->panel_lists;
    if (lists.empty()) lists.resize(1);
    if (!lists[0].landed) STORM_HIP_TRY(hipEventCreateWithFlags(&lists[0].landed, hipEventDisableTiming));
    STORM_HIP_TRY(hipEventRecord(lists[0].landed, ctx->stream));
    STORM_HIP_TRY(hipStreamWaitEvent(ctx->copy_stream, lists[0].landed, 0));
    std::vector<uint64_t> first_tile;
    {
        const uint64_t n = std::max<uint64_t>(1, std::min<uint64_t>(8, tiles / 4));
        for (uint64_t p = 0; p <= n; ++p) first_tile.push_back(tiles * p / n);
    }
    const uint64_t n_panels = first_tile.size() - 1;
    const uint32_t n_kslices2 = 2u * ((m->n_words + 7u) / 8u);
    if (lists.size() < n_panels) lists.resize(n_panels);
    ctx->pass_report[0] |= STORM_HIP_RAN_BIT_STRIPS;
    ctx->pass_report[1] += ranges_word_pairs({{0, m->n_rows}}, (uint64_t)n_kslices2 * 4u, 1);
    ctx->k2_operands_used = 5;
    ctx->k2_strip_rows_used = 64;
    uint64_t n_total = 0;
    for (uint64_t p = 0; p < n_panels; ++p) {
        const uint64_t t0 = first_tile[p], t1 = first_tile[p + 1];
        if (t0 >= t1) continue;
        const uint64_t row0 = t0 * kStripATile, row1 = std::min<uint64_t>(m->n_rows, t1 * kStripATile);
        PanelList& l = lists[p];
        if (!l.landed) STORM_HIP_TRY(hipEventCreateWithFlags(&l.landed, hipEventDisableTiming));
        STORM_HIP_TRY(hipMemcpy2DAsync(m->d + row0 * m->stride_words, pitch, host_rows + row0 * src_stride_words,
                                       src_stride_words * 8, (size_t)m->n_words * 8, row1 - row0, hipMemcpyHostToDevice,
                                       ctx->copy_stream));
        STORM_HIP_TRY(hipEventRecord(l.landed, ctx->copy_stream));
        StripOptions po = strip_options_of(ctx, 2);
        po.max_run = 128;
        po.shard_pairs = po.persistent = po.one_slice_probe = 0;
        RowRange rg{0, row1};
        rg.back_from = row0;
        const std::vector<RowRange> panel = {rg};
        const StripRequest rq = strip_request(po, panel, n_kslices2, 0, 1, (uint32_t)kStripATile);
        if (!l.list.holds(rq)) {
            std::vector<StripItem> items;
            uint32_t qb[8], qc[8];
            plan_strips(rq, panel, items, qb, qc);
            if (items.size() >= (1ull << 31)) {
                set_error("pairw_dense_upload: %zu strip items exceed the grid limit", items.size());
                return STORM_HIP_EINVAL;
            }
            if (int rc = l.list.put(ctx, rq, items.data(), items.size(), "pairw_dense_upload: a panel's strip items", 1024 * sizeof(StripItem)))
                return rc;
        }
        STORM_HIP_TRY(hipStreamWaitEvent(ctx->stream, l.landed, 0));
        if (l.list.n) {
            hipLaunchKernelGGL(strip16_bits_kernel, dim3(l.list.n), dim3(kStripThreads), (size_t)ctx->k2_lds_pad, ctx->stream,
                               reinterpret_cast<const uint8_t*>(m->d), pitch, l.list.recs(), ctx->d_slots,
                               (unsigned long long*)nullptr, (uint32_t)kSlots);
            STORM_HIP_TRY(hipGetLastError());
        }
        n_total += l.list.n;
    }
    ctx->last_info[0] = n_total;
    ctx->last_info[1] = ctx->k2_stages_per_item;
    ctx->last_info[2] = 1;
    ctx->last_info[3] = n_panels;
    return launch_fold_slots(ctx, d_total);
}

int strip_operands_of(const storm_hip_ctx_t* ctx) {
    if (ctx->k2_strip_operands == 6) return 5;
    if (ctx->k2_strip_operands != 0) return ctx->k2_strip_operands;
    return (ctx->k2_ring == kStripRingDefault && ctx->k2_shape == 16) ? 5 : 4;
}
int launch_pairw_mfma(storm_hip_ctx_t* ctx, const storm_hip_matrix_s* m, uint32_t shard_rank,
                      uint32_t shard_count, uint64_t* d_total) {
    const int strip_mode = ctx->variant == 5 ? 2 : ctx->variant == 4 ? 1 : 0;
    const int operands = strip_operands_of(ctx);
    if (strip_mode == 1 && (operands == 1 || operands == 2 || operands == 3 || operands == 5) && !ctx->k2_persistent && ctx->k2_debug == 0 &&
        (m->n_rows + kStripATile - 1) / kStripATile * kStripATile <= m->n_rows_pad &&
        m->stride_words * 8 * (uint64_t)kStripBRows < (1ull << 32))
    {
        const bool wide = operands == 5 && ctx->k2_strip_operands == 6 && (m->n_rows + 511u) / 512u * 512u <= m->n_rows_pad;
        ctx->k2_operands_used = wide ? 6 : operands;
        return launch_pairw_bits(ctx, m, shard_rank, shard_count, wide ? 6 : operands, d_total);
    }
    ctx->k2_operands_used = 4;
    const uint64_t tile = strip_mode == 2 ? 512 : kStripATile;
    const uint64_t n_rows4 = (m->n_rows + tile - 1) / tile * tile;
    std::vector<RowRange> ranges;
    if (m->n_rows > 1) ranges.push_back({0, m->n_rows});
    return launch_pairw_mfma_ranges(ctx, m->d, m->stride_words, m->n_rows_pad, n_rows4, ranges,
                                    shard_rank, shard_count, strip_mode, d_total, m->generation,
                                    m->n_words);
}

}

#ifdef STORM_HIP_PROBES
extern "C" int storm_hip_probe_clock(uint64_t out[3]) {
    unsigned long long v[4] = {0, 0, 0, 0};
    if (hipDeviceSynchronize() != hipSuccess) return STORM_HIP_EINVAL;
    if (hipMemcpyFromSymbol(v, HIP_SYMBOL(storm::g_clock_probe), sizeof(v)) != hipSuccess) return STORM_HIP_EINVAL;
    out[0] = v[0];
    out[1] = v[1];
    out[2] = v[2];
    const unsigned long long z[4] = {0, 0, 0, 0};
    if (hipMemcpyToSymbol(HIP_SYMBOL(storm::g_clock_probe), z, sizeof(z)) != hipSuccess) return STORM_HIP_EINVAL;
    return STORM_HIP_OK;
}
#endif
```

### stormbitmaps_amd/csrc/storm_hip_plan.cpp

```cpp
#include "storm_hip_plan.h"

#include <algorithm>
#include <cmath>
#include <cstdio>
#include <cstdlib>
#include <chrono>
#include <exception>

#include "storm_hip.h"

namespace storm {

bool timing_env() {
    static const bool on = getenv("STORM_HIP_TIMING") != nullptr;
    return on;
}

uint64_t ranges_hash(const std::vector<RowRange>& ranges) {
    uint64_t h = 1469598103934665603ull;
    for (const RowRange& r : ranges) {
        h = (h ^ r.r0) * 1099511628211ull;
        h = (h ^ r.r1) * 1099511628211ull;
        h = (h ^ r.a_end) * 1099511628211ull;
        h = (h ^ r.back_from) * 1099511628211ull;
    }
    return h;
}

int plan_tile_sum(const TileSumRequest& rq, const std::vector<RowRange>& ranges, std::vector<MfmaItem>& items) {
    const uint32_t total_stages = rq.total_stages, shard_rank = rq.shard_rank, shard_count = rq.shard_count;
    const uint32_t spi = std::max(1u, rq.stages_per_item);
    const bool diag_only = rq.diag_only != 0;
    std::vector<std::pair<uint16_t, uint16_t>> tiles;
    for (const RowRange& rg : ranges) {
        const uint32_t b0 = (uint32_t)(rg.r0 / kTile);
        const uint32_t nT = (uint32_t)((rg.r1 - rg.r0 + kTile - 1) / kTile);
        const uint32_t nTa = rg.a_end ? (uint32_t)std::min<uint64_t>(nT, (std::min(rg.a_end, rg.r1) - rg.r0 + kTile - 1) / kTile) : nT;
        for (uint32_t gi = 0; gi < nTa; gi += 4)
            for (uint32_t gj = gi / 8 * 8; gj < nT; gj += 8)
                for (uint32_t i = gi; i < std::min(gi + 4, nTa); ++i)
                    for (uint32_t j = std::max(gj, i); j < std::min(gj + 8, nT); ++j)
                        if (!diag_only || i == j)
                            tiles.emplace_back((uint16_t)(b0 + i), (uint16_t)(b0 + j));
    }
    std::vector<std::pair<uint32_t, uint32_t>> slices;
    for (uint32_t g0 = 0; g0 < total_stages; g0 += kGroupStages) {
        if ((g0 / kGroupStages) % shard_count != shard_rank) continue;
        const uint32_t g1 = std::min(total_stages, g0 + kGroupStages);
        for (uint32_t s0 = g0; s0 < g1; s0 += spi) slices.emplace_back(s0, std::min(spi, g1 - s0));
    }
    items.clear();
    const size_t n = tiles.size();
    for (const auto& sl : slices) {
        const uint32_t s0 = sl.first, ns = sl.second;
        for (size_t c = 0; c < n; c += 256)
            for (size_t pos = 0; pos < 32; ++pos)
                for (size_t x = 0; x < 8; ++x) {
                    const size_t L = c + x * 32 + pos;
                    if (L >= n) continue;
                    if (rq.one_tile_probe)
                        items.push_back({tiles[0].first, tiles[0].first, s0, ns});
                    else
                        items.push_back({tiles[L].first, tiles[L].second, s0, ns});
                }
    }
    if (items.size() != slices.size() * n) {
        set_error("K2 item table construction lost tiles (%zu != %zu)", items.size(),
                  slices.size() * n);
        return STORM_HIP_EINVAL;
    }
    if (items.size() >= (1ull << 31)) {
        set_error("K2: %zu tile items exceed the grid limit", items.size());
        return STORM_HIP_EINVAL;
    }
    return STORM_HIP_OK;
}

static inline uint32_t strip_item_cost(const StripItem& it, uint32_t per_tile) {
    return (it.j1 - it.j0) + it.diag * per_tile + 10u;
}

struct StripShaping {
    int max_run = 128, tail_run = 32, tail_slices = 3, lpt_rounds = 6;
    int xcd_group = 1;
    bool persistent = false, one_slice_probe = false;
    bool pair_space = false;
};
static void build_strip_items(const StripShaping& sh, const std::vector<RowRange>& ranges,
                              uint32_t n_kslices, uint32_t shard_rank, uint32_t shard_count,
                              uint32_t a_tile, std::vector<StripItem>& items,
                              uint32_t queue_base[8], uint32_t queue_count[8], double* makespan = nullptr,
                              uint32_t slots_per_xcd = 128) {
    const uint32_t kMaxRun = (uint32_t)std::min(4096, std::max(1, sh.max_run));
    const uint32_t kTailRun = (uint32_t)std::min(4096, std::max(1, sh.tail_run));
    const uint32_t kPerTile = a_tile / kStripBRows;
    std::vector<std::vector<uint32_t>> slices_of(8);
    uint32_t local = 0;
    const bool pair_mode = sh.pair_space && shard_count > 1;
    const uint32_t modulo_slices = pair_mode ? n_kslices : strip_modulo_slices(n_kslices, shard_count);
    const uint32_t xg = (uint32_t)std::max(1, sh.xcd_group);
    for (uint32_t ks = 0; ks < modulo_slices; ++ks)
        if (pair_mode || strip_owns_slice(ks, shard_rank, shard_count)) slices_of[(local++ / xg) % 8].push_back(ks);
    std::vector<uint64_t> pair_load(shard_count, 0);
    auto emit_slice_all = [&](uint32_t ks, uint32_t max_run, std::vector<StripItem>& dst) {
        const uint32_t ks_data = sh.one_slice_probe ? ks % 8u : ks;
        for (const RowRange& rg : ranges) {
            if (rg.back_from != ~0ull) {
                const uint32_t blk0 = (uint32_t)(rg.r0 / kStripBRows);
                for (uint64_t a0 = rg.back_from; a0 < rg.r1; a0 += a_tile) {
                    const uint32_t a_row0 = (uint32_t)a0, end = (uint32_t)(a0 / kStripBRows);
                    if (end <= blk0) {
                        dst.push_back({a_row0, 1, end, end, ks_data});
                        continue;
                    }
                    for (uint32_t j0 = blk0; j0 < end; j0 += max_run)
                        dst.push_back({a_row0, (uint32_t)(j0 == blk0), j0, std::min(end, j0 + max_run), ks_data});
                }
                continue;
            }
            const uint64_t a_rows = (rg.a_end ? std::min(rg.a_end, rg.r1) : rg.r1) - rg.r0;
            const uint32_t nA = (uint32_t)((a_rows + a_tile - 1) / a_tile);
            const uint32_t jend = (uint32_t)((rg.r1 + kStripBRows - 1) / kStripBRows);
            for (uint32_t i = 0; i < nA; ++i) {
                const uint32_t a_row0 = (uint32_t)rg.r0 + i * a_tile;
                const uint32_t first = a_row0 / (uint32_t)kStripBRows + kPerTile;
                if (first >= jend) {
                    dst.push_back({a_row0, 1, first, first, ks_data});
                    continue;
                }
                for (uint32_t j0 = first; j0 < jend; j0 += max_run)
                    dst.push_back({a_row0, (uint32_t)(j0 == first), j0,
                                   std::min(jend, j0 + max_run), ks_data});
            }
        }
    };
    const uint32_t kTailLen = std::min(kMaxRun, kTailRun);
    std::vector<StripItem> proto_main, proto_tail;
    bool have_main = false, have_tail = false;
    auto by_length = [&](const StripItem& p, const StripItem& q) {
        return (p.j1 - p.j0) + p.diag * kPerTile > (q.j1 - q.j0) + q.diag * kPerTile;
    };
    auto emit_copy = [&](uint32_t ks, uint32_t max_run, std::vector<StripItem>& dst) {
        std::vector<StripItem>& proto = max_run == kMaxRun ? proto_main : proto_tail;
        bool& have = max_run == kMaxRun ? have_main : have_tail;
        if (!have) {
            emit_slice_all(0u, max_run, proto);
            if (max_run == kMaxRun) std::stable_sort(proto.begin(), proto.end(), by_length);
            have = true;
        }
        const uint32_t ks_data = sh.one_slice_probe ? ks % 8u : ks;
        const size_t at = dst.size();
        dst.insert(dst.end(), proto.begin(), proto.end());
        for (size_t k = at; k < dst.size(); ++k) dst[k].ks = ks_data;
    };
    auto emit_slice = [&](uint32_t ks, uint32_t max_run, std::vector<StripItem>& dst) {
        if (!pair_mode) return (max_run == kMaxRun || max_run == kTailLen) ? emit_copy(ks, max_run, dst) : emit_slice_all(ks, max_run, dst);
        std::vector<StripItem> all;
        emit_slice_all(ks, max_run, all);
        std::stable_sort(all.begin(), all.end(), [&](const StripItem& p, const StripItem& q) {
            return strip_item_cost(p, kPerTile) > strip_item_cost(q, kPerTile);
        });
        for (const StripItem& it : all) {
            const uint32_t r = (uint32_t)(std::min_element(pair_load.begin(), pair_load.end()) - pair_load.begin());
            pair_load[r] += strip_item_cost(it, kPerTile);
            if (r == shard_rank) dst.push_back(it);
        }
    };
    std::vector<std::vector<StripItem>> leftover_of(8);
    if (modulo_slices < n_kslices) {
        std::vector<uint64_t> load(shard_count, 0);
        for (uint32_t ks = modulo_slices; ks < n_kslices; ++ks) {
            std::vector<StripItem> all;
            emit_slice_all(ks, std::min(kMaxRun, kTailRun), all);
            std::stable_sort(all.begin(), all.end(), [&](const StripItem& p, const StripItem& q) {
                return strip_item_cost(p, kPerTile) > strip_item_cost(q, kPerTile);
            });
            const uint32_t xcd = (local++ / xg) % 8;
            for (const StripItem& it : all) {
                const uint32_t r = (uint32_t)(std::min_element(load.begin(), load.end()) - load.begin());
                load[r] += strip_item_cost(it, kPerTile);
                if (r == shard_rank) leftover_of[xcd].push_back(it);
            }
        }
    }
    const uint32_t kTail = (uint32_t)std::max(0, sh.tail_slices);
    std::vector<std::vector<StripItem>> per_xcd(8);
    const int n_lists = makespan ? 1 : 8;
    for (int x = 0; x < n_lists; ++x) {
        const std::vector<uint32_t>& sl = slices_of[x];
        const size_t n_main = sl.size() > kTail ? sl.size() - kTail : 0;
        for (size_t k = 0; k < n_main; ++k) {
            if (!pair_mode) {
                emit_slice(sl[k], kMaxRun, per_xcd[x]);
                continue;
            }
            std::vector<StripItem> one;
            emit_slice(sl[k], kMaxRun, one);
            std::stable_sort(one.begin(), one.end(), by_length);
            per_xcd[x].insert(per_xcd[x].end(), one.begin(), one.end());
        }
        std::vector<StripItem> tail;
        for (size_t k = n_main; k < sl.size(); ++k) emit_slice(sl[k], std::min(kMaxRun, kTailRun), tail);
        tail.insert(tail.end(), leftover_of[x].begin(), leftover_of[x].end());
        std::stable_sort(tail.begin(), tail.end(), [&](const StripItem& p, const StripItem& q) {
            return (p.j1 - p.j0) + p.diag * kPerTile > (q.j1 - q.j0) + q.diag * kPerTile;
        });
        per_xcd[x].insert(per_xcd[x].end(), tail.begin(), tail.end());
        if (per_xcd[x].size() <= (size_t)128 * (size_t)std::max(0, sh.lpt_rounds))
            std::stable_sort(per_xcd[x].begin(), per_xcd[x].end(),
                             [&](const StripItem& p, const StripItem& q) {
                                 return (p.j1 - p.j0) + p.diag * kPerTile > (q.j1 - q.j0) + q.diag * kPerTile;
                             });
    }
    if (makespan) {
        auto cost_of = [&](const StripItem& it) { return (double)(it.j1 - it.j0) + (it.diag ? kPerTile + 3.0 : 0.0) + 5.0; };
        const std::vector<StripItem>& list = per_xcd[0];
        const size_t n_slots = std::max<uint32_t>(1, slots_per_xcd);
        const size_t start = list.size() > 16 * n_slots ? list.size() - 16 * n_slots : 0;
        double before = 0;
        for (size_t k = 0; k < start; ++k) before += cost_of(list[k]);
        std::vector<double> slot(n_slots, before / (double)n_slots);
        auto later = [](double p, double q) { return p > q; };
        for (size_t k = start; k < list.size(); ++k) {
            std::pop_heap(slot.begin(), slot.end(), later);
            slot.back() += cost_of(list[k]);
            std::push_heap(slot.begin(), slot.end(), later);
        }
        const double worst = *std::max_element(slot.begin(), slot.end());
        *makespan = worst;
        items.clear();
        return;
    }
    items.clear();
    if (sh.persistent) {
        for (int x = 0; x < 8; ++x) {
            queue_base[x] = (uint32_t)items.size();
            queue_count[x] = (uint32_t)per_xcd[x].size();
            items.insert(items.end(), per_xcd[x].begin(), per_xcd[x].end());
        }
    } else {
        size_t longest = 0;
        for (auto& v : per_xcd) longest = std::max(longest, v.size());
        for (size_t pos = 0; pos < longest; ++pos)
            for (int x = 0; x < 8; ++x)
                if (pos < per_xcd[x].size()) items.push_back(per_xcd[x][pos]);
    }
}

static StripShaping choose_strip_shaping(const StripOptions& o, const std::vector<RowRange>& ranges, uint32_t n_kslices,
                                         uint32_t shard_count, uint32_t a_tile) {
    StripShaping sh;
    sh.tail_run = o.tail_run;
    sh.tail_slices = o.tail_slices;
    sh.lpt_rounds = o.lpt_rounds;
    sh.xcd_group = o.xcd_group;
    sh.persistent = o.persistent != 0;
    sh.one_slice_probe = o.one_slice_probe != 0;
    sh.pair_space = o.shard_pairs != 0;
    sh.max_run = o.max_run;
    if (o.max_run != 0) return sh;
    const uint32_t slots = (uint32_t)std::max(1, o.n_cus / 8 * 4);
    const bool timing = timing_env();
    double best = 0;
    for (int cand : {96, 64, 128}) {
        StripShaping trial = sh;
        trial.max_run = cand;
        double worst = 0;
        size_t n_items = 0;
        for (uint32_t r = 0; r < shard_count; ++r) {
            std::vector<StripItem> tmp;
            uint32_t qb[8], qc[8];
            double ms = 0;
            build_strip_items(trial, ranges, n_kslices, r, shard_count, a_tile, tmp, qb, qc, &ms, slots);
            worst = std::max(worst, ms);
            n_items += tmp.size();
        }
        if (timing)
            fprintf(stderr, "[strip plan] max_run %3d: %zu items over %u rank(s), predicted makespan %.0f stages\n", cand,
                    n_items, shard_count, worst);
        if (sh.max_run == 0 || worst < best * 0.995) {
            sh.max_run = cand;
            best = worst;
        }
    }
    return sh;
}

StripRequest strip_request(const StripOptions& opt, const std::vector<RowRange>& ranges, uint32_t n_kslices,
                           uint32_t shard_rank, uint32_t shard_count, uint32_t a_tile) {
    StripRequest rq;
    rq.opt = opt;
    rq.n_kslices = n_kslices;
    rq.shard_rank = shard_rank;
    rq.shard_count = shard_count;
    rq.a_tile = a_tile;
    rq.ranges_hash = ranges_hash(ranges);
    return rq;
}

void plan_strips(const StripRequest& rq, const std::vector<RowRange>& ranges, std::vector<StripItem>& items,
                 uint32_t queue_base[8], uint32_t queue_count[8], int* run_chosen) {
    const StripShaping sh = choose_strip_shaping(rq.opt, ranges, rq.n_kslices, rq.shard_count, rq.a_tile);
    if (run_chosen) *run_chosen = sh.max_run;
    build_strip_items(sh, ranges, rq.n_kslices, rq.shard_rank, rq.shard_count, rq.a_tile, items, queue_base, queue_count);
}

void xcd_grouped_tiles(uint32_t i0, uint32_t i1, uint32_t j0, uint32_t j1, bool triangle,
                              std::vector<std::pair<uint16_t, uint16_t>>& out) {
    std::vector<std::vector<std::pair<uint16_t, uint16_t>>> per_xcd(8);
    uint32_t g = 0;
    for (uint32_t gi = i0; gi < i1; gi += 4)
        for (uint32_t gj = triangle ? std::max(j0, gi / 8 * 8) : j0; gj < j1; gj += 8) {
            std::vector<std::pair<uint16_t, uint16_t>>& dst = per_xcd[g % 8];
            const size_t before = dst.size();
            for (uint32_t i = gi; i < std::min(gi + 4, i1); ++i)
                for (uint32_t j = std::max(gj, triangle ? i + 1 : gj); j < std::min(gj + 8, j1); ++j)
                    dst.emplace_back((uint16_t)i, (uint16_t)j);
            if (dst.size() != before) ++g;
        }
    size_t longest = 0;
    for (auto& v : per_xcd) longest = std::max(longest, v.size());
    for (size_t pos = 0; pos < longest; ++pos)
        for (int x = 0; x < 8; ++x)
            if (pos < per_xcd[x].size()) out.push_back(per_xcd[x][pos]);
}

void plan_matrix_tiles(const MatrixTilesRequest& rq, std::vector<MfmaItem>& items, MatrixPlan* plan) {
    const std::vector<std::pair<uint16_t, uint16_t>>& tiles = rq.tiles;
    const uint32_t total_stages = rq.total_stages;
    const size_t slots = (size_t)std::max(1u, rq.n_cus);
    size_t leftover = rq.split ? tiles.size() % slots : 0;
    constexpr uint32_t kMaxExactStages = (1u << 24) / 128u - 1u;
    uint32_t min_parts = 1;
    if (total_stages > kMaxExactStages) {
        leftover = tiles.size();
        min_parts = (total_stages + kMaxExactStages - 1) / kMaxExactStages;
    }
    const size_t n_full = tiles.size() - leftover;
    const uint32_t max_parts = std::max(min_parts, total_stages / (uint32_t)rq.min_part);
    auto cost_of = [&](size_t t) { return rq.cost.empty() ? 1.0f : std::max(0.05f, rq.cost[t]); };
    double left_cost = 0;
    for (size_t t = n_full; t < tiles.size(); ++t) left_cost += cost_of(t);
    const double per_part = left_cost / (double)slots;
    std::vector<uint32_t> parts_of(leftover, 1);
    size_t n_parts = 0;
    for (size_t t = n_full; t < tiles.size(); ++t) {
        const double want = per_part > 0 ? cost_of(t) / per_part : 1.0;
        n_parts += parts_of[t - n_full] = std::min(max_parts, std::max(min_parts, (uint32_t)want));
    }
    while (min_parts == 1 && n_parts < slots && leftover > 0) {
        size_t best = leftover;
        double longest = 0;
        for (size_t i = 0; i < leftover; ++i) {
            const double len = cost_of(n_full + i) / parts_of[i];
            if (parts_of[i] < max_parts && len > longest) longest = len, best = i;
        }
        if (best == leftover) break;
        ++parts_of[best];
        ++n_parts;
    }
    items.clear();
    for (size_t t = 0; t < n_full; ++t) items.push_back({tiles[t].first, tiles[t].second, 0, total_stages});
    for (size_t t = n_full; t < tiles.size(); ++t) {
        const uint32_t parts = parts_of[t - n_full];
        for (uint32_t p = 0; p < parts; ++p) {
            const uint32_t s0 = (uint32_t)((uint64_t)(total_stages / 4) * p / parts) * 4u;
            const uint32_t s1 = (uint32_t)((uint64_t)(total_stages / 4) * (p + 1) / parts) * 4u;
            items.push_back({tiles[t].first, tiles[t].second, s0, s1 - s0});
        }
    }
    plan->n_items = (uint32_t)items.size();
    plan->n_full = (uint32_t)n_full;
    plan->n_cut = (uint32_t)leftover;
    for (size_t t = n_full; t < tiles.size(); ++t) items.push_back({tiles[t].first, tiles[t].second, 0u, 0u});
}

void plan_tile128(const Tile128Request& rq, Tile128Plan* plan) {
    const uint32_t ia0 = rq.ia0, ia1 = rq.ia1, jb0 = rq.jb0, jb1 = rq.jb1, total_stages = rq.total_stages, n_cus = rq.n_cus;
    const bool triangle = rq.triangle != 0, narrow_windows = rq.narrow_windows != 0;
    const int slots_per_cu = rq.slots_per_cu, diag_cost_pct = rq.diag_cost_pct;
    int min_chunks = rq.min_chunks;
    struct T { uint16_t I, J; bool diag; };
    std::vector<T> tiles;
    for (int pass = 0; pass < 2; ++pass)
        for (uint32_t gi = ia0; gi < ia1; gi += 4)
            for (uint32_t gj = jb0; gj < jb1; gj += 8)
                for (uint32_t i = gi; i < std::min(gi + 4, ia1); ++i)
                    for (uint32_t j = gj; j < std::min(gj + 8, jb1); ++j) {
                        if (triangle && j < i) continue;
                        if (triangle && rq.lag && (uint64_t)j > ((uint64_t)kThTile * i + kThTile - 1u + rq.lag) / kThTile) continue;
                        const bool diag = triangle && j == i;
                        if (diag != (pass == 1)) continue;
                        tiles.push_back({(uint16_t)i, (uint16_t)j, diag});
                    }
    const uint32_t nC = total_stages / 4u;
    plan->n_tiles = (uint32_t)tiles.size();
    plan->n_windows = 0;
    plan->items.clear();
    if (tiles.empty() || nC == 0) return;
    const uint32_t weight = std::max(rq.chunk_weight, 1u);
    const uint32_t kMaxExactChunks = ((1u << 24) - 1u) / weight;
    const uint32_t max_narrow_chunks = 65535u / weight;
    constexpr double kItemChunks = 5.0;
    min_chunks = std::max(min_chunks, (int)(nC / 32000u) + 1);
    const uint32_t min_parts = (nC + kMaxExactChunks - 1) / kMaxExactChunks;
    const uint32_t max_parts = std::max(min_parts, nC / (uint32_t)min_chunks);
    const size_t nT = tiles.size();
    std::vector<uint32_t> parts_of(nT), best_parts;
    double best_load = 0;
    for (int spc = 1; spc <= 2; ++spc) {
        if (slots_per_cu > 0 && spc != slots_per_cu) continue;
        const size_t slots = (size_t)n_cus * spc;
        const double dcost = spc >= 2 ? diag_cost_pct / 100.0 : 1.0;
        auto cost_of = [&](size_t t) { return tiles[t].diag ? dcost : 1.0; };
        const size_t n_whole = min_parts > 1 ? 0 : nT / slots * slots;
        std::fill(parts_of.begin(), parts_of.end(), 1u);
        double rest = 0;
        for (size_t t = n_whole; t < nT; ++t) rest += cost_of(t) * nC;
        const double seg = rest / (double)slots;
        size_t n_items = n_whole;
        for (size_t t = n_whole; t < nT; ++t)
            n_items += parts_of[t] = std::min(max_parts, std::max(min_parts, (uint32_t)(cost_of(t) * nC / std::max(seg, 1e-9))));
        while (n_items < n_whole + slots) {
            size_t best = nT;
            double longest = 0;
            for (size_t t = n_whole; t < nT; ++t) {
                const double len = cost_of(t) * nC / parts_of[t];
                if (parts_of[t] < max_parts && len > longest) longest = len, best = t;
            }
            if (best == nT) break;
            ++parts_of[best];
            ++n_items;
        }
        double longest = 0;
        for (size_t t = n_whole; t < nT; ++t) longest = std::max(longest, cost_of(t) * std::ceil((double)nC / parts_of[t]));
        const double load = spc * ((double)(n_whole / slots) * nC + longest) + kItemChunks * (double)n_items / n_cus;
        if (best_parts.empty() || load < best_load) best_load = load, best_parts = parts_of;
    }
    for (uint32_t t = 0; t < nT; ++t) {
        const uint32_t np = best_parts[t];
        const uint16_t narrow = (np > 1 && (nC + np - 1) / np <= max_narrow_chunks && narrow_windows) ? kThNarrow : (uint16_t)0;
        for (uint32_t p = 0; p < np; ++p) {
            const uint32_t c0 = (uint32_t)((uint64_t)nC * p / np), c1 = (uint32_t)((uint64_t)nC * (p + 1) / np);
            plan->items.push_back({tiles[t].I, tiles[t].J, c0 * 4u, (c1 - c0) * 4u, t, np > 1 ? plan->n_windows : 0u,
                                   (uint16_t)((uint16_t)p | narrow), (uint16_t)np});
        }
        if (np > 1) plan->n_windows += np;
    }
    std::stable_sort(plan->items.begin(), plan->items.end(),
                     [](const PartItem& a, const PartItem& b) { return a.n_stages > b.n_stages; });
}

BitstreamRequest bitstream_request(const BitstreamShaping& sh, const std::vector<RowRange>& ranges, uint32_t n_kslices,
                                   uint32_t shard_rank, uint32_t shard_count, uint32_t n_cus, uint64_t pitch_bytes) {
    return {sh, n_kslices, shard_rank, shard_count, n_cus, pitch_bytes, ranges_hash(ranges)};
}
// ... 593 lines not shown

}

static int export_part_items(const char* who, const storm::Tile128Plan& plan, uint32_t* out, uint64_t capacity_items,
                             uint64_t* n_items) {
    using namespace storm;
    *n_items = plan.items.size();
    if (out) {
        if (capacity_items < plan.items.size()) {
            set_error("%s: capacity %llu < %zu items", who, (unsigned long long)capacity_items, plan.items.size());
            return STORM_HIP_EINVAL;
        }
        for (size_t k = 0; k < plan.items.size(); ++k) {
            const PartItem& it = plan.items[k];
            uint32_t* o = out + 8 * k;
            o[0] = it.I, o[1] = it.J, o[2] = it.stage0 / 4u, o[3] = it.n_stages / 4u, o[4] = it.tile;
            o[5] = (uint32_t)(it.part & (uint16_t)~kThNarrow), o[6] = it.n_parts, o[7] = (it.part & kThNarrow) ? 1u : 0u;
        }
    }
    return STORM_HIP_OK;
}

extern "C" int storm_hip_matrix_plan(uint64_t n_rows_a, uint64_t n_rows_b, uint32_t n_words, uint64_t band_row0,
                                     uint64_t band_rows, uint32_t n_cus, int slots_per_cu, int min_chunks, int diag_cost_pct,
                                     uint32_t* out, uint64_t capacity_items, uint64_t* n_items) {
    using namespace storm;
    if (!n_items || n_rows_a == 0 || n_words == 0 || n_cus == 0 || slots_per_cu < 0 || slots_per_cu > 2 || min_chunks < 1 ||
        diag_cost_pct < 10 || diag_cost_pct > 100) {
        set_error("matrix_plan: bad arguments");
        return STORM_HIP_EINVAL;
    }
    try {
        const uint32_t total_stages = (n_words + 7u) / 8u * 4u;
        Tile128Plan plan;
        if (n_rows_b == 0) {
            const uint64_t end = std::min(n_rows_a, band_row0 + (band_rows ? band_rows : n_rows_a));
            if (band_row0 < end)
                plan_tile128({(uint32_t)(band_row0 / kThTile), (uint32_t)((end + kThTile - 1) / kThTile), 0u,
                              (uint32_t)((n_rows_a + kThTile - 1) / kThTile), 1u, total_stages, n_cus, slots_per_cu, min_chunks,
                              diag_cost_pct, 1u, 0u, kThWeightBits}, &plan);
        } else {
            const uint64_t rows_a = (n_rows_a + kTile - 1) / kTile * kTile;
            plan_tile128({0u, (uint32_t)((n_rows_a + kThTile - 1) / kThTile), (uint32_t)(rows_a / kThTile),
                          (uint32_t)((rows_a + n_rows_b + kThTile - 1) / kThTile), 0u, total_stages, n_cus, slots_per_cu,
                          min_chunks, diag_cost_pct, 1u, 0u, kThWeightBits}, &plan);
        }
        return export_part_items("matrix_plan", plan, out, capacity_items, n_items);
    } catch (const std::exception& e) {
        set_error("matrix_plan: %s", e.what());
        return STORM_HIP_ENOMEM;
    }
}

extern "C" int storm_hip_dosage_plan(uint64_t n_rows_a, uint64_t n_rows_b, uint32_t n_words, uint64_t band_row0,
                                     uint64_t band_rows, uint32_t n_cus, int slots_per_cu, int min_chunks, int diag_cost_pct,
                                     uint32_t* out, uint64_t capacity_items, uint64_t* n_items) {
    using namespace storm;
    if (!n_items || n_rows_a == 0 || n_rows_b != 0 || n_words == 0 || n_cus == 0 || slots_per_cu < 0 || slots_per_cu > 2 ||
        min_chunks < 1 || diag_cost_pct < 10 || diag_cost_pct > 100 || (n_rows_a + kThTile - 1) / kThTile > 65535u) {
        set_error("dosage_plan: bad arguments (the dosage form is the triangle of one matrix: n_rows_b must be 0)");
        return STORM_HIP_EINVAL;
    }
    try {
        Tile128Plan plan;
        const uint64_t end = std::min(n_rows_a, band_row0 + std::min(band_rows ? band_rows : n_rows_a, n_rows_a));
        if (band_row0 < end)
            plan_tile128({(uint32_t)(band_row0 / kThTile), (uint32_t)((end + kThTile - 1) / kThTile), 0u,
                          (uint32_t)((n_rows_a + kThTile - 1) / kThTile), 1u, (n_words + 7u) / 8u * 4u, n_cus, slots_per_cu,
                          min_chunks, diag_cost_pct, 1u, 0u, kThWeightDosage}, &plan);
        return export_part_items("dosage_plan", plan, out, capacity_items, n_items);
    } catch (const std::exception& e) {
        set_error("dosage_plan: %s", e.what());
        return STORM_HIP_ENOMEM;
    }
}

extern "C" int storm_hip_dosage_square_plan(uint64_t n_rows_a, uint64_t n_rows_b, uint32_t n_words, uint32_t n_cus,
                                            int slots_per_cu, int min_chunks, int diag_cost_pct, uint32_t* out,
                                            uint64_t capacity_items, uint64_t* n_items) {
    using namespace storm;
    const uint64_t rows_a = (n_rows_a + kTile - 1) / kTile * kTile;
    if (!n_items || n_rows_a == 0 || n_rows_b == 0 || n_words == 0 || n_cus == 0 || slots_per_cu < 0 || slots_per_cu > 2 ||
        min_chunks < 1 || diag_cost_pct < 10 || diag_cost_pct > 100 || n_rows_a > (1ull << 32) || n_rows_b > (1ull << 32) ||
        (rows_a + n_rows_b + kThTile - 1) / kThTile > 65535u) {
        set_error("dosage_square_plan: bad arguments");
        return STORM_HIP_EINVAL;
    }
    try {
        Tile128Plan plan;
        plan_tile128({0u, (uint32_t)((n_rows_a + kThTile - 1) / kThTile), (uint32_t)(rows_a / kThTile),
                      (uint32_t)((rows_a + n_rows_b + kThTile - 1) / kThTile), 0u, (n_words + 7u) / 8u * 4u, n_cus, slots_per_cu,
                      min_chunks, diag_cost_pct, 1u, 0u, kThWeightDosage}, &plan);
        return export_part_items("dosage_square_plan", plan, out, capacity_items, n_items);
    } catch (const std::exception& e) {
        set_error("dosage_square_plan: %s", e.what());
        return STORM_HIP_ENOMEM;
    }
}

extern "C" int storm_hip_lag_plan(uint64_t n_rows, uint32_t n_words, uint64_t max_lag, uint64_t band_row0, uint64_t band_rows,
                                  uint32_t n_cus, int slots_per_cu, int min_chunks, int diag_cost_pct, uint32_t* out,
                                  uint64_t capacity_items, uint64_t* n_items) {
    using namespace storm;
    if (!n_items || n_rows == 0 || n_words == 0 || max_lag == 0 || n_cus == 0 || slots_per_cu < 0 || slots_per_cu > 2 ||
        min_chunks < 1 || diag_cost_pct < 10 || diag_cost_pct > 100 || (n_rows + kThTile - 1) / kThTile > 65535u) {
        set_error("lag_plan: bad arguments");
        return STORM_HIP_EINVAL;
    }
    try {
        Tile128Plan plan;
        const uint64_t end = std::min(n_rows, band_row0 + std::min(band_rows ? band_rows : n_rows, n_rows));
        const uint32_t lag = (uint32_t)std::min<uint64_t>(max_lag, n_rows - 1);
        if (band_row0 < end && lag)
            plan_tile128({(uint32_t)(band_row0 / kThTile), (uint32_t)((end + kThTile - 1) / kThTile), 0u,
                          (uint32_t)((n_rows + kThTile - 1) / kThTile), 1u, (n_words + 7u) / 8u * 4u, n_cus, slots_per_cu,
                          min_chunks, diag_cost_pct, 1u, lag, kThWeightBits}, &plan);
        return export_part_items("lag_plan", plan, out, capacity_items, n_items);
    } catch (const std::exception& e) {
        set_error("lag_plan: %s", e.what());
        return STORM_HIP_ENOMEM;
    }
}

extern "C" int storm_hip_lag_dosage_plan(uint64_t n_rows, uint32_t n_words, uint64_t max_lag, uint64_t band_row0,
                                         uint64_t band_rows, uint32_t n_cus, int slots_per_cu, int min_chunks, int diag_cost_pct,
                                         uint32_t* out, uint64_t capacity_items, uint64_t* n_items) {
    using namespace storm;
    if (!n_items || n_rows == 0 || n_words == 0 || max_lag == 0 || n_cus == 0 || slots_per_cu < 0 || slots_per_cu > 2 ||
        min_chunks < 1 || diag_cost_pct < 10 || diag_cost_pct > 100 || (n_rows + kThTile - 1) / kThTile > 65535u) {
        set_error("lag_dosage_plan: bad arguments");
        return STORM_HIP_EINVAL;
    }
    try {
        Tile128Plan plan;
        const uint64_t end = std::min(n_rows, band_row0 + std::min(band_rows ? band_rows : n_rows, n_rows));
        const uint32_t lag = (uint32_t)std::min<uint64_t>(max_lag, n_rows - 1);
        if (band_row0 < end && lag)
            plan_tile128({(uint32_t)(band_row0 / kThTile), (uint32_t)((end + kThTile - 1) / kThTile), 0u,
                          (uint32_t)((n_rows + kThTile - 1) / kThTile), 1u, (n_words + 7u) / 8u * 4u, n_cus, slots_per_cu,
                          min_chunks, diag_cost_pct, 1u, lag, kThWeightDosage}, &plan);
        return export_part_items("lag_dosage_plan", plan, out, capacity_items, n_items);
    } catch (const std::exception& e) {
        set_error("lag_dosage_plan: %s", e.what());
        return STORM_HIP_ENOMEM;
    }
}

extern "C" int storm_hip_strip_plan3(uint64_t n_rows, uint32_t n_words, uint32_t shard_rank,
                                     uint32_t shard_count, int form, int pair_space, int max_run, int tail_run,
                                     int tail_slices, int lpt_rounds, uint32_t n_cus, uint32_t* out,
                                     uint64_t capacity_items, uint64_t* n_items, int* run_chosen) {
    using namespace storm;
    if (!n_items || shard_count == 0 || shard_rank >= shard_count || n_words == 0 || form < 0 || form > 2 ||
        max_run < 0 || max_run > 4096 || tail_run < 1 || tail_run > 4096 || tail_slices < 0 || tail_slices > 255 ||
        lpt_rounds < 0 || lpt_rounds > 63 || n_cus == 0) {
        set_error("strip_plan: bad arguments");
        return STORM_HIP_EINVAL;
    }
    try {
        const uint32_t n_kslices = form == 0 ? (n_words + 3u) / 4u : form == 1 ? 2u * ((n_words + 7u) / 8u) : strip_rows_kslices(n_words);
        std::vector<RowRange> ranges;
        if (n_rows > 1) ranges.push_back({0, n_rows});
        std::vector<StripItem> items;
        uint32_t qb[8], qc[8];
        StripOptions o;
        o.max_run = max_run;
        o.tail_run = tail_run;
        o.tail_slices = tail_slices;
        o.lpt_rounds = lpt_rounds;
        o.shard_pairs = pair_space != 0;
        o.n_cus = (int)n_cus;
        o.xcd_group = form == 0 ? 1 : form == 1 ? 2 : (int)kStripRowsXcdGroup;
        plan_strips(strip_request(o, ranges, n_kslices, shard_rank, shard_count, form == 2 ? kStripRowsATile : (uint32_t)kStripATile),
                    ranges, items, qb, qc, run_chosen);
        *n_items = items.size();
        if (out)
            for (uint64_t i = 0; i < std::min<uint64_t>(capacity_items, items.size()); ++i) {
                out[i * 5 + 0] = items[i].a_row0;
                out[i * 5 + 1] = items[i].diag;
                out[i * 5 + 2] = items[i].j0;
                out[i * 5 + 3] = items[i].j1;
                out[i * 5 + 4] = items[i].ks;
            }
    } catch (const std::exception& e) {
        set_error("strip_plan: %s", e.what());
        return STORM_HIP_ENOMEM;
    }
    return STORM_HIP_OK;
}

extern "C" int storm_hip_strip_plan2(uint64_t n_rows, uint32_t n_words, uint32_t shard_rank,
                                     uint32_t shard_count, int form, int pair_space, uint32_t* out,
                                     uint64_t capacity_items, uint64_t* n_items) {
    const storm::StripOptions d;
    return storm_hip_strip_plan3(n_rows, n_words, shard_rank, shard_count, form, pair_space, d.max_run, d.tail_run,
                                 d.tail_slices, d.lpt_rounds, (uint32_t)d.n_cus, out, capacity_items, n_items, nullptr);
}

extern "C" int storm_hip_strip_plan(uint64_t n_rows, uint32_t n_words, uint32_t shard_rank,
                                    uint32_t shard_count, uint32_t* out, uint64_t capacity_items,
                                    uint64_t* n_items) {
    return storm_hip_strip_plan2(n_rows, n_words, shard_rank, shard_count, 0, 0, out, capacity_items, n_items);
}

extern "C" int storm_hip_stream_plan(uint64_t n_rows, uint32_t n_words, uint32_t shard_rank, uint32_t shard_count,
                                     uint32_t n_cus, uint32_t* out, uint64_t capacity_segments,
                                     uint64_t* n_segments, uint32_t* n_workgroups) {
    using namespace storm;
    if (!n_segments || shard_count == 0 || shard_rank >= shard_count || n_words == 0 || n_cus == 0) {
        set_error("stream_plan: bad arguments");
        return STORM_HIP_EINVAL;
    }
    try {
        std::vector<RowRange> ranges;
        if (n_rows > 1) ranges.push_back({0, n_rows});
        BitstreamPlan plan;
        const uint64_t stride_words = ((uint64_t)n_words + kChunkWords - 1) / kChunkWords * kChunkWords;
        build_bitstream(bitstream_request(BitstreamShaping{}, ranges, (n_words + 7u) / 8u, shard_rank, shard_count, n_cus,
                                          stride_words * 8),
                        ranges, plan);
        *n_segments = plan.segs.size();
        if (n_workgroups) *n_workgroups = plan.groups;
        if (out) {
            uint32_t wg = 0;
            for (uint64_t i = 0; i < std::min<uint64_t>(capacity_segments, plan.segs.size()); ++i) {
                while (wg + 1 < plan.first.size() && plan.first[wg + 1] <= i) ++wg;
                const BitSeg& sg = plan.segs[i];
                uint32_t* o = out + i * 8;
                o[0] = wg;
                o[1] = sg.a_blk;
                o[2] = sg.ks;
                o[3] = sg.b_first;
                o[4] = sg.n_b;
                o[5] = sg.range_nb;
                o[6] = sg.flags & kBsDiag;
                o[7] = 4u + sg.n_b;
            }
        }
    } catch (const std::exception& e) {
        set_error("stream_plan: %s", e.what());
        return STORM_HIP_ENOMEM;
    }
    return STORM_HIP_OK;
}
```

### stormbitmaps_amd/csrc/storm_hip_plan.h

```cpp
#pragma once

#include <cstdint>
#include <cstring>
#include <type_traits>
#include <utility>
#include <vector>

namespace storm {

void set_error(const char* fmt, ...);
bool timing_env();

template <class T>
inline bool same_request(const T& a, const T& b) {
    static_assert(std::has_unique_object_representations_v<T>, "a request struct with padding cannot be compared with memcmp");
    return !memcmp(&a, &b, sizeof(T));
}

constexpr int kChunkWords = 64;

constexpr int kTile = 256;
constexpr int kStageBytes = 64;
constexpr uint32_t kGroupStages = 32;

struct MfmaItem {
    uint16_t I, J;
    uint32_t stage0;
    uint32_t n_stages;
};
static_assert(sizeof(MfmaItem) == 12, "read by device code");

constexpr uint32_t kOwnSlices = 4;
constexpr int kStripRowBytes = 128;
constexpr int kStripBRows = 64;
constexpr int kStripWaves = 4;
constexpr int kStripATile = 64 * kStripWaves;
constexpr uint32_t kStripRowsATile = 512;
constexpr uint32_t kStripRowsXcdGroup = 8;
inline uint32_t strip_rows_kslices(uint32_t n_words) { return (n_words + 1u) / 2u; }
constexpr uint32_t kStripRowsBlocks = kStripRowsATile / (uint32_t)kStripBRows;
constexpr uint32_t kStripRowsWaves = 4;
enum StripRowsRole : uint32_t { kStripRowsSkip = 0, kStripRowsOwn = 1, kStripRowsWhole = 2 };
constexpr uint32_t strip_rows_block(uint32_t wave, uint32_t half) { return half ? kStripRowsBlocks - 1u - wave : wave; }
constexpr StripRowsRole strip_rows_role(uint32_t wave, uint32_t half, uint32_t d) {
    return d < strip_rows_block(wave, half) ? kStripRowsSkip : d == strip_rows_block(wave, half) ? kStripRowsOwn : kStripRowsWhole;
}
constexpr uint32_t strip_rows_diag_begin(uint32_t wave) {
    return strip_rows_block(wave, 0) < strip_rows_block(wave, 1) ? strip_rows_block(wave, 0) : strip_rows_block(wave, 1);
}
constexpr uint32_t strip_rows_diag_end(uint32_t) { return kStripRowsBlocks; }
constexpr uint32_t strip_rows_role_mfmas(StripRowsRole r) { return r == kStripRowsWhole ? 16u : r == kStripRowsOwn ? 10u : 0u; }
static_assert(strip_rows_block(0, 0) < strip_rows_block(0, 1) && strip_rows_block(1, 0) < strip_rows_block(1, 1) &&
              strip_rows_block(2, 0) < strip_rows_block(2, 1) && strip_rows_block(3, 0) < strip_rows_block(3, 1),
              "strip16_rows_kernel walks the low half's own block first");

constexpr uint32_t kStripRowsNoTrim = 0xFFFFFFFFu;
constexpr uint32_t strip_rows_real_frags(uint32_t blk, uint32_t n_rows) {
    const uint32_t row0 = blk * (uint32_t)kStripBRows;
    return n_rows <= row0 ? 0u : n_rows - row0 >= (uint32_t)kStripBRows ? 4u : (n_rows - row0 + 15u) / 16u;
}
constexpr uint32_t strip_rows_real_blocks(uint32_t a_row0, uint32_t n_rows) {
    return n_rows <= a_row0 ? 0u : n_rows - a_row0 >= kStripRowsATile ? kStripRowsBlocks
                                                                     : (n_rows - a_row0 + (uint32_t)kStripBRows - 1u) / (uint32_t)kStripBRows;
}
constexpr bool strip_rows_top_trimmed(uint32_t j0, uint32_t j1, uint32_t n_rows) {
    return j1 > j0 && strip_rows_real_frags(j1 - 1u, n_rows) - 1u < 2u;
}
constexpr uint32_t strip_rows_item_mfmas(uint32_t a_row0, uint32_t diag, uint32_t j0, uint32_t j1, uint32_t n_rows) {
    const uint32_t T = j1 - j0;
    uint32_t n = strip_rows_top_trimmed(j0, j1, n_rows)
                     ? kStripRowsWaves * 8u * (4u * (T - 1u) + strip_rows_real_frags(j1 - 1u, n_rows))
                     : kStripRowsWaves * 8u * 4u * T;
    if (diag) {
        const uint32_t nb = strip_rows_real_blocks(a_row0, n_rows);
        for (uint32_t w = 0; w < kStripRowsWaves; ++w)
            for (uint32_t half = 0; half < 2u; ++half)
                for (uint32_t d = 0; d < nb; ++d)
                    if (strip_rows_block(w, half) < nb) n += strip_rows_role_mfmas(strip_rows_role(w, half, d));
    }
    return n;
}

struct StripItem {
    uint32_t a_row0;
    uint32_t diag;
    uint32_t j0, j1;
    uint32_t ks;
};
static_assert(sizeof(StripItem) == 20, "read by device code");

struct BitSeg {
    uint32_t a_blk;
    uint32_t ks;
    uint32_t b_first;
    uint32_t n_b;
    uint32_t range_b0;
    uint32_t range_nb;
    uint32_t flags;
    uint32_t pad;
};
static_assert(sizeof(BitSeg) == 32, "read by device code");
constexpr uint32_t kBsDiag = 1u;
constexpr uint32_t kBsMaxStages = 8192;

constexpr uint32_t kThTile = 128u;
struct PartItem {
    uint16_t I, J;
    uint32_t stage0, n_stages;
    uint32_t tile;
    uint32_t win0;
    uint16_t part, n_parts;
};
static_assert(sizeof(PartItem) == 24, "read by device code");
constexpr uint16_t kThNarrow = 0x8000u;
constexpr uint32_t kThWeightBits = 512u;
constexpr uint32_t kThWeightDosage = 9u * 256u;

struct RowRange {
    uint64_t r0, r1;
    uint64_t a_end = 0;
    uint64_t back_from = ~0ull;
};
uint64_t ranges_hash(const std::vector<RowRange>& ranges);

inline uint32_t strip_modulo_slices(uint32_t n_kslices, uint32_t shard_count) {
    return n_kslices / kOwnSlices / shard_count * shard_count * kOwnSlices;
}
inline bool strip_owns_slice(uint32_t ks, uint32_t shard_rank, uint32_t shard_count) {
    return (ks / kOwnSlices) % shard_count == shard_rank;
}

struct TileSumRequest {
    uint64_t ranges_hash;
    uint32_t total_stages, shard_rank, shard_count;
    uint32_t stages_per_item;
    uint32_t diag_only;
    uint32_t one_tile_probe;
    bool operator==(const TileSumRequest& o) const { return same_request(*this, o); }
};
int plan_tile_sum(const TileSumRequest& rq, const std::vector<RowRange>& ranges, std::vector<MfmaItem>& items);

struct StripOptions {
    int32_t max_run = 0, tail_run = 32, tail_slices = 3, lpt_rounds = 6;
    int32_t shard_pairs = 0;
    int32_t n_cus = 256;
    int32_t xcd_group = 1;
    int32_t persistent = 0;
    int32_t one_slice_probe = 0;
};
struct StripRequest {
    StripOptions opt;
    uint32_t n_kslices, shard_rank, shard_count, a_tile;
    uint32_t unused = 0;
    uint64_t ranges_hash;
    bool operator==(const StripRequest& o) const { return same_request(*this, o); }
};
StripRequest strip_request(const StripOptions& opt, const std::vector<RowRange>& ranges, uint32_t n_kslices,
                           uint32_t shard_rank, uint32_t shard_count, uint32_t a_tile);
void plan_strips(const StripRequest& rq, const std::vector<RowRange>& ranges, std::vector<StripItem>& items,
                 uint32_t queue_base[8], uint32_t queue_count[8], int* run_chosen = nullptr);

void xcd_grouped_tiles(uint32_t i0, uint32_t i1, uint32_t j0, uint32_t j1, bool triangle,
                       std::vector<std::pair<uint16_t, uint16_t>>& out);
struct MatrixTilesRequest {
    std::vector<std::pair<uint16_t, uint16_t>> tiles;
    std::vector<float> cost;
    uint32_t total_stages = 0;
    uint32_t n_cus = 1;
    int32_t split = 1;
    int32_t min_part = 32;
    bool operator==(const MatrixTilesRequest& o) const {
        return total_stages == o.total_stages && n_cus == o.n_cus && split == o.split && min_part == o.min_part &&
               tiles == o.tiles && cost == o.cost;
    }
};
struct MatrixPlan {
    uint32_t n_items = 0;
    uint32_t n_full = 0;
    uint32_t n_cut = 0;
};
void plan_matrix_tiles(const MatrixTilesRequest& rq, std::vector<MfmaItem>& items, MatrixPlan* plan);

struct Tile128Request {
    uint32_t ia0, ia1, jb0, jb1;
    uint32_t triangle;
    uint32_t total_stages;
    uint32_t n_cus;
    int32_t slots_per_cu, min_chunks, diag_cost_pct;
    uint32_t narrow_windows;
    uint32_t lag;
    uint32_t chunk_weight;
    bool operator==(const Tile128Request& o) const { return same_request(*this, o); }
};
struct Tile128Plan {
    std::vector<PartItem> items;
    uint32_t n_tiles = 0, n_windows = 0;
};
void plan_tile128(const Tile128Request& rq, Tile128Plan* plan);

struct BitstreamShaping {
    int32_t groups_per_cu = 0;
    int32_t min_piece = 6;
    int32_t min_run = 2;
    int32_t long_piece = 80;
    int32_t w3_1 = 120, w3_2 = 60;
    int32_t weighted_min = 16;
    int32_t single_round_max = 220;
};
struct BitstreamRequest {
    BitstreamShaping sh;
    uint32_t n_kslices, shard_rank, shard_count, n_cus;
    uint64_t pitch_bytes;
    uint64_t ranges_hash;
    bool operator==(const BitstreamRequest& o) const { return same_request(*this, o); }
};
struct BitstreamPlan {
    std::vector<BitSeg> segs;
    std::vector<uint32_t> bases;
    std::vector<uint32_t> first_stage;
    std::vector<uint32_t> first;
    uint32_t groups = 0;
    uint64_t stages = 0;
    uint32_t max_stages = 0;
};
BitstreamRequest bitstream_request(const BitstreamShaping& sh, const std::vector<RowRange>& ranges, uint32_t n_kslices,
                                   uint32_t shard_rank, uint32_t shard_count, uint32_t n_cus, uint64_t pitch_bytes);
void build_bitstream(const BitstreamRequest& rq, const std::vector<RowRange>& ranges, BitstreamPlan& plan);

constexpr uint32_t kBlockWords = 1024;
constexpr uint32_t kMaxBlockId = 65536;
constexpr int kABlockRows = 128;
constexpr uint32_t kProbeRows = 128;
constexpr uint32_t kProbeOctBits = 13;
constexpr uint32_t kProbeOctants = 1u << (16 - kProbeOctBits);
constexpr uint32_t kFatGroups = 4;

struct Seg {
    uint32_t a_row0;
    uint32_t a_end;
    uint32_t j_lo;
    uint32_t j_hi;
};
static_assert(sizeof(Seg) == 16, "read by device code");

struct ProbeItem {
    uint32_t a_begin, a_end;
    uint32_t n_begin, n_end;
    uint32_t b_begin, b_end;
    uint32_t a0;
};
static_assert(sizeof(ProbeItem) == 28, "read by device code");
struct ProbeFatItem {
    uint32_t at[kFatGroups + 1];
    uint32_t b_begin, b_end;
    uint32_t first;
};
static_assert(sizeof(ProbeFatItem) == 32, "read by device code");
struct ProbeRegion { uint32_t e_begin, e_end, pool_row0, octant; };
static_assert(sizeof(ProbeRegion) == 16, "read by device code");

struct ArenaBlocks {
    uint64_t n_rows = 0, n_blocks = 0;
    const uint64_t* row_block_offset = nullptr;
    const uint32_t* block_id = nullptr;
    const uint8_t* block_kind = nullptr;
    const uint32_t* block_n = nullptr;
    const void* const* block_ptr = nullptr;
};

struct ArenaLaps {
    int64_t t0_ns;
    ArenaLaps();
    void lap(const char* what);
};

struct ArenaColumns {
    std::vector<RowRange> cols;
    uint64_t census[4] = {0, 0, 0, 0};
    uint64_t n_pool_rows = 0;
    uint64_t pool_rows_ready = 0;
    std::vector<uint64_t> col_list0;
    std::vector<uint8_t> col_probe;
    std::vector<uint32_t> col_avg_len;
};
struct ArenaRows {
    std::vector<uint32_t> list_row, list_len, dense_row;
    std::vector<uint64_t> list_blk, dense_blk;
    std::vector<uint64_t> probe_blocks;
    std::vector<int64_t> col_entry;
};
int plan_arena_columns(const ArenaBlocks& in, ArenaColumns* cols, ArenaRows* rows, ArenaLaps& laps);

struct ProbeWork {
    std::vector<ProbeRegion> probe_regions;
    std::vector<ProbeItem> items;
    std::vector<uint32_t> item_col;
    std::vector<ProbeFatItem> fat_items;
    std::vector<uint32_t> fat_col;
};
struct ProbeLayout {
    size_t n_probe_elems = 0;
    std::vector<uint32_t> run_dst;
    std::vector<uint32_t> block_local;
    std::vector<uint32_t> atoms;
};
int plan_arena_probe(const ArenaBlocks& in, const ArenaColumns& cols, const ArenaRows& rows, const std::vector<uint32_t>& run_end,
                     ProbeWork* work, ProbeLayout* layout, ArenaLaps& laps);

struct ProbeLaunchRequest {
    uint32_t shard_rank = 0, shard_count = 0;
    int32_t bundle = 0;
    std::vector<uint8_t> use_probe;
    bool operator==(const ProbeLaunchRequest& o) const {
// ... 32 lines not shown
```

### stormbitmaps_amd/dist.py

```python
from __future__ import annotations

import os
from typing import Callable, Tuple


def rank_world() -> Tuple[int, int, int]:
    return (int(os.environ.get("RANK", "0")), int(os.environ.get("WORLD_SIZE", "1")),
            int(os.environ.get("LOCAL_RANK", "0")))


def free_port() -> int:
    import socket
    with socket.socket() as sock:
        sock.bind(("127.0.0.1", 0))
        return sock.getsockname()[1]


def init_process_group(backend: str):
    import torch.distributed as dist
    if not dist.is_initialized():
        rank, world, _ = rank_world()
        os.environ.setdefault("MASTER_ADDR", "127.0.0.1")
        if "MASTER_PORT" not in os.environ:
            if world > 1:
                raise RuntimeError("MASTER_PORT is not set: start the ranks with torch.distributed.run "
                                   "or `python bench.py --gpus N`, which pick a free rendezvous port")
            os.environ["MASTER_PORT"] = str(free_port())
        dist.init_process_group(backend=backend, rank=rank, world_size=world)
    return dist


def strip_plan(n_rows: int, n_words: int, rank: int, world: int, form: int = 1, pair_space: int = 0, *,
               max_run: int = 0, tail_run: int = 32, tail_slices: int = 3, lpt_rounds: int = 6, n_cus: int = 256,
               return_run: bool = False):
    import ctypes as C

    import numpy as np

    from . import _lib
    lib = _lib.load()
    n = C.c_uint64(0)
    run = C.c_int(0)
    args = (n_rows, n_words, rank, world, form, pair_space, max_run, tail_run, tail_slices, lpt_rounds, n_cus)
    _lib.check(lib.storm_hip_strip_plan3(*args, None, 0, C.byref(n), C.byref(run)), "storm_hip_strip_plan3")
    out = np.zeros((int(n.value), 5), dtype=np.uint32)
    if n.value:
        _lib.check(lib.storm_hip_strip_plan3(*args, out.ctypes.data_as(C.c_void_p), n.value, C.byref(n), C.byref(run)),
                   "storm_hip_strip_plan3")
    return (out, int(run.value)) if return_run else out


def slice_columns(mat, ks: int, form: int = 1):
    import numpy as np
    if form == 0:
        return np.ascontiguousarray(mat[:, 4 * ks:4 * ks + 4])
    if form == 2:
        return np.ascontiguousarray(mat[:, 2 * ks:2 * ks + 2])
    c = ks // 2
    mask = np.uint64(0xCCCCCCCCCCCCCCCC if ks & 1 else 0x3333333333333333)
    return np.ascontiguousarray(mat[:, 8 * c:8 * c + 8] & mask)


def stream_plan(n_rows: int, n_words: int, rank: int = 0, world: int = 1, n_cus: int = 256):
    import ctypes as C

    import numpy as np

    from . import _lib
    lib = _lib.load()
    n, g = C.c_uint64(0), C.c_uint32(0)
    _lib.check(lib.storm_hip_stream_plan(n_rows, n_words, rank, world, n_cus, None, 0, C.byref(n), C.byref(g)),
               "storm_hip_stream_plan")
    out = np.zeros((int(n.value), 8), dtype=np.uint32)
    if n.value:
        _lib.check(lib.storm_hip_stream_plan(n_rows, n_words, rank, world, n_cus, out.ctypes.data_as(C.c_void_p),
                                             n.value, C.byref(n), C.byref(g)), "storm_hip_stream_plan")
    return out, int(g.value)


def matrix_plan(n_rows_a: int, n_words: int, n_rows_b: int = 0, band_row0: int = 0, band_rows: int = 0, n_cus: int = 256,
                slots_per_cu: int = 0, min_chunks: int = 8, diag_cost_pct: int = 80):
    import ctypes as C

    import numpy as np

    from . import _lib
    lib = _lib.load()
    n = C.c_uint64(0)
    args = (n_rows_a, n_rows_b, n_words, band_row0, band_rows, n_cus, slots_per_cu, min_chunks, diag_cost_pct)
    _lib.check(lib.storm_hip_matrix_plan(*args, None, 0, C.byref(n)), "storm_hip_matrix_plan")
    out = np.zeros((int(n.value), 8), dtype=np.uint32)
    if n.value:
        _lib.check(lib.storm_hip_matrix_plan(*args, out.ctypes.data_as(C.c_void_p), n.value, C.byref(n)),
                   "storm_hip_matrix_plan")
    return out


def dosage_plan(n_rows: int, n_words: int, n_cus: int = 256, slots_per_cu: int = 0, min_chunks: int = 8, diag_cost_pct: int = 80):
    import ctypes as C

    import numpy as np

    from . import _lib
    lib = _lib.load()
    n = C.c_uint64(0)
    args = (n_rows, 0, n_words, 0, 0, n_cus, slots_per_cu, min_chunks, diag_cost_pct)
    _lib.check(lib.storm_hip_dosage_plan(*args, None, 0, C.byref(n)), "storm_hip_dosage_plan")
    out = np.zeros((int(n.value), 8), dtype=np.uint32)
    if n.value:
        _lib.check(lib.storm_hip_dosage_plan(*args, out.ctypes.data_as(C.c_void_p), n.value, C.byref(n)),
                   "storm_hip_dosage_plan")
    return out


def dosage_square_plan(n_rows_a: int, n_rows_b: int, n_words: int, n_cus: int = 256, slots_per_cu: int = 0, min_chunks: int = 8,
                       diag_cost_pct: int = 80):
    import ctypes as C

    import numpy as np

    from . import _lib
    lib = _lib.load()
    n = C.c_uint64(0)
    args = (n_rows_a, n_rows_b, n_words, n_cus, slots_per_cu, min_chunks, diag_cost_pct)
    _lib.check(lib.storm_hip_dosage_square_plan(*args, None, 0, C.byref(n)), "storm_hip_dosage_square_plan")
    out = np.zeros((int(n.value), 8), dtype=np.uint32)
    if n.value:
        _lib.check(lib.storm_hip_dosage_square_plan(*args, out.ctypes.data_as(C.c_void_p), n.value, C.byref(n)),
                   "storm_hip_dosage_square_plan")
    return out


def lag_plan(n_rows: int, n_words: int, max_lag: int, band_row0: int = 0, band_rows: int = 0, n_cus: int = 256,
             slots_per_cu: int = 0, min_chunks: int = 8, diag_cost_pct: int = 80):
    import ctypes as C

    import numpy as np

    from . import _lib
    lib = _lib.load()
    n = C.c_uint64(0)
    args = (n_rows, n_words, max_lag, band_row0, band_rows, n_cus, slots_per_cu, min_chunks, diag_cost_pct)
    _lib.check(lib.storm_hip_lag_plan(*args, None, 0, C.byref(n)), "storm_hip_lag_plan")
    out = np.zeros((int(n.value), 8), dtype=np.uint32)
    if n.value:
        _lib.check(lib.storm_hip_lag_plan(*args, out.ctypes.data_as(C.c_void_p), n.value, C.byref(n)), "storm_hip_lag_plan")
    return out


def lag_dosage_plan(n_rows: int, n_words: int, max_lag: int, band_row0: int = 0, band_rows: int = 0, n_cus: int = 256,
                    slots_per_cu: int = 0, min_chunks: int = 8, diag_cost_pct: int = 80):
    import ctypes as C

    import numpy as np

    from . import _lib
    lib = _lib.load()
    n = C.c_uint64(0)
    args = (n_rows, n_words, max_lag, band_row0, band_rows, n_cus, slots_per_cu, min_chunks, diag_cost_pct)
    _lib.check(lib.storm_hip_lag_dosage_plan(*args, None, 0, C.byref(n)), "storm_hip_lag_dosage_plan")
    out = np.zeros((int(n.value), 8), dtype=np.uint32)
    if n.value:
        _lib.check(lib.storm_hip_lag_dosage_plan(*args, out.ctypes.data_as(C.c_void_p), n.value, C.byref(n)),
                   "storm_hip_lag_dosage_plan")
    return out


def allreduce_total(partial: int, device=None) -> int:
    import torch
    import torch.distributed as dist
    if partial >= 1 << 63:
        raise OverflowError("partial total does not fit the int64 all-reduce transport")
    t = torch.tensor([partial], dtype=torch.int64, device=device)
    if dist.is_initialized() and dist.get_world_size() > 1:
        dist.all_reduce(t, op=dist.ReduceOp.SUM)
    return int(t.item())


def sharded_pairw(partial_fn: Callable[[int, int], int], device=None) -> int:
    import torch.distributed as dist
    rank, world = (dist.get_rank(), dist.get_world_size()) if dist.is_initialized() else (0, 1)
    return allreduce_total(partial_fn(rank, world), device=device)
```

Before: 147200 billion words/s.

## Auto-select strip tail shaping via makespan model and MFMA-based item costs for rows form

For the 128-rows-per-wave strip form, the planner now sorts items longest-first by an MFMA-count cost that accounts for row trimming and diagonal blocks, rather than by run length. When the user has not set tail options, it also simulates per-CU slot scheduling for several candidate (max_run, tail_run, tail_slices) shapings and picks the one with the lowest modeled makespan. The goal is better load balance at the end of the kernel. The cost is more host-side planning work and reliance on a model that may not match hardware behaviour.

```diff
diff --git a/stormbitmaps_amd/csrc/storm_hip.hip b/stormbitmaps_amd/csrc/storm_hip.hip
--- a/stormbitmaps_amd/csrc/storm_hip.hip
+++ b/stormbitmaps_amd/csrc/storm_hip.hip
@@ -560,6 +560,7 @@
     void (*after)(storm_hip_ctx_t* ctx, int64_t value);
 };
 
+static void tail_is_set(storm_hip_ctx_t* ctx, int64_t) { ctx->k2_tail_set = 1; }
 static void drop_shadow(storm_hip_ctx_t* ctx, int64_t) { memset(ctx->x4_key, 0, sizeof(ctx->x4_key)); }
 static void restart_series(storm_hip_ctx_t* ctx, int64_t value) {
     if (value == 1) ctx->kernel_events_used = 0;
@@ -661,8 +662,8 @@
         {"k2_persistent", &C::k2_persistent, BOOL, 0, 0, 0, {}, nullptr, {1},
          "k2_persistent (strip_fp4_kernel with work queues) is a form of the tools build (`make probes`), not of the shipped library"},
         {"k2_lpt_rounds", &C::k2_lpt_rounds, RANGE, 0, 63, 0, {}, "k2_lpt_rounds must be 0..63"},
-        {"k2_tail_slices", &C::k2_tail_slices, RANGE, 0, 255, 0, {}, "k2_tail_slices must be 0..255"},
-        {"k2_tail_run", &C::k2_tail_run, RANGE, 1, 4096, 0, {}, "k2_tail_run must be 1..4096"},
+        {"k2_tail_slices", &C::k2_tail_slices, RANGE, 0, 255, 0, {}, "k2_tail_slices must be 0..255", {}, nullptr, nullptr, tail_is_set},
+        {"k2_tail_run", &C::k2_tail_run, RANGE, 1, 4096, 0, {}, "k2_tail_run must be 1..4096", {}, nullptr, nullptr, tail_is_set},
         {"k2_debug", &C::k2_debug, HOOK, 0, 0, 0, {}, nullptr, {}, nullptr, set_debug},
         {"time_kernels", &C::time_kernels, BOOL, 0, 0, 0, {}, nullptr, {}, nullptr, nullptr, restart_series},
         {"chunks_per_item", &C::chunks_per_item, RANGE, 0, 4096, 0, {}, "chunks_per_item out of range"},
@@ -713,6 +714,9 @@
     if (!strcmp(key, "k2_operands_used")) return ctx->k2_operands_used;
     if (!strcmp(key, "k2_strip_rows_used")) return ctx->k2_strip_rows_used;
     if (!strcmp(key, "k2_tile_shape_used")) return ctx->k2_tile_shape_eff;
+    if (!strcmp(key, "k2_max_run_used")) return ctx->k2_max_run_used;
+    if (!strcmp(key, "k2_tail_run_used")) return ctx->k2_tail_run_used;
+    if (!strcmp(key, "k2_tail_slices_used")) return ctx->k2_tail_slices_used;
     if (!strcmp(key, "n_cus")) return ctx->n_cus;
     if (!strcmp(key, "probes_build") || !strcmp(key, "probes_built")) return kToolsBuild;
     return -1;
diff --git a/stormbitmaps_amd/csrc/storm_hip_internal.h b/stormbitmaps_amd/csrc/storm_hip_internal.h
--- a/stormbitmaps_amd/csrc/storm_hip_internal.h
+++ b/stormbitmaps_amd/csrc/storm_hip_internal.h
@@ -225,6 +225,8 @@
     int k2_lpt_rounds = 6;
     int k2_tail_slices = 3;
     int k2_tail_run = 32;
+    int k2_tail_set = 0;
+    int k2_max_run_used = 0, k2_tail_run_used = 0, k2_tail_slices_used = 0;
     int time_kernels = 0;
     std::vector<hipEvent_t> kernel_events;
     size_t kernel_events_used = 0;
diff --git a/stormbitmaps_amd/csrc/storm_hip_mfma.hip b/stormbitmaps_amd/csrc/storm_hip_mfma.hip
--- a/stormbitmaps_amd/csrc/storm_hip_mfma.hip
+++ b/stormbitmaps_amd/csrc/storm_hip_mfma.hip
@@ -1186,11 +1186,13 @@
     return ctx->items.put(ctx, rq, items.data(), items.size(), "K2: the item table", kItemsFloorBytes);
 }
 
-static StripOptions strip_options_of(const storm_hip_ctx_t* ctx, int xcd_group) {
+static StripOptions strip_options_of(const storm_hip_ctx_t* ctx, int xcd_group, bool rows_form) {
     StripOptions o;
     o.max_run = ctx->k2_max_run;
     o.tail_run = ctx->k2_tail_run;
     o.tail_slices = ctx->k2_tail_slices;
+    o.rows_form = rows_form;
+    o.tail_auto = rows_form && !ctx->k2_tail_set;
     o.lpt_rounds = ctx->k2_lpt_rounds;
     o.shard_pairs = ctx->k2_shard_pairs != 0;
     o.n_cus = ctx->n_cus;
@@ -1202,12 +1204,16 @@
 
 static int ensure_strip_items(storm_hip_ctx_t* ctx, const std::vector<RowRange>& ranges,
                               uint32_t n_kslices, uint32_t shard_rank, uint32_t shard_count,
-                              uint32_t a_tile, int xcd_group = 1) {
-    const StripRequest rq = strip_request(strip_options_of(ctx, xcd_group), ranges, n_kslices, shard_rank, shard_count, a_tile);
+                              uint32_t a_tile, int xcd_group = 1, bool rows_form = false) {
+    const StripRequest rq = strip_request(strip_options_of(ctx, xcd_group, rows_form), ranges, n_kslices, shard_rank, shard_count, a_tile);
     if (ctx->strips.holds(rq)) return STORM_HIP_OK;
     ctx->strips.forget();
     std::vector<StripItem> items;
-    plan_strips(rq, ranges, items, ctx->strips.queue_base, ctx->strips.queue_count);
+    StripChoice used;
+    plan_strips(rq, ranges, items, ctx->strips.queue_base, ctx->strips.queue_count, &used);
+    ctx->k2_max_run_used = used.max_run;
+    ctx->k2_tail_run_used = used.tail_run;
+    ctx->k2_tail_slices_used = used.tail_slices;
     if (items.size() >= (1ull << 31)) {
         set_error("K2s: %zu strip items exceed the grid limit", items.size());
         return STORM_HIP_EINVAL;
@@ -1906,7 +1912,7 @@
         set_error("K2b: the 128-rows-per-wave form takes A tiles of 512 rows");
         return STORM_HIP_EINVAL;
     }
-    if (int rc = ensure_strip_items(ctx, ranges, n_kslices2, shard_rank, shard_count, a_tile, rows128 ? (int)kStripRowsXcdGroup : 2))
+    if (int rc = ensure_strip_items(ctx, ranges, n_kslices2, shard_rank, shard_count, a_tile, rows128 ? (int)kStripRowsXcdGroup : 2, rows128))
         return rc;
     const uint32_t n_strip = ctx->strips.n;
     const uint32_t waves = rows128 ? 4u : a_tile / (uint32_t)kStripBRows;
@@ -2055,7 +2061,7 @@
                                        src_stride_words * 8, (size_t)m->n_words * 8, row1 - row0, hipMemcpyHostToDevice,
                                        ctx->copy_stream));
         STORM_HIP_TRY(hipEventRecord(l.landed, ctx->copy_stream));
-        StripOptions po = strip_options_of(ctx, 2);
+        StripOptions po = strip_options_of(ctx, 2, false);
         po.max_run = 128;
         po.shard_pairs = po.persistent = po.one_slice_probe = 0;
         RowRange rg{0, row1};
diff --git a/stormbitmaps_amd/csrc/storm_hip_plan.cpp b/stormbitmaps_amd/csrc/storm_hip_plan.cpp
--- a/stormbitmaps_amd/csrc/storm_hip_plan.cpp
+++ b/stormbitmaps_amd/csrc/storm_hip_plan.cpp
@@ -85,7 +85,42 @@
     int xcd_group = 1;
     bool persistent = false, one_slice_probe = false;
     bool pair_space = false;
+    bool rows_cost = false;
+    uint32_t n_rows = kStripRowsNoTrim;
 };
+static void emit_strip_slice(const std::vector<RowRange>& ranges, uint32_t a_tile, uint32_t ks_data, uint32_t max_run,
+                             std::vector<StripItem>& dst) {
+    const uint32_t kPerTile = a_tile / kStripBRows;
+    for (const RowRange& rg : ranges) {
+        if (rg.back_from != ~0ull) {
+            const uint32_t blk0 = (uint32_t)(rg.r0 / kStripBRows);
+            for (uint64_t a0 = rg.back_from; a0 < rg.r1; a0 += a_tile) {
+                const uint32_t a_row0 = (uint32_t)a0, end = (uint32_t)(a0 / kStripBRows);
+                if (end <= blk0) {
+                    dst.push_back({a_row0, 1, end, end, ks_data});
+                    continue;
+                }
+                for (uint32_t j0 = blk0; j0 < end; j0 += max_run)
+                    dst.push_back({a_row0, (uint32_t)(j0 == blk0), j0, std::min(end, j0 + max_run), ks_data});
+            }
+            continue;
+        }
+        const uint64_t a_rows = (rg.a_end ? std::min(rg.a_end, rg.r1) : rg.r1) - rg.r0;
+        const uint32_t nA = (uint32_t)((a_rows + a_tile - 1) / a_tile);
+        const uint32_t jend = (uint32_t)((rg.r1 + kStripBRows - 1) / kStripBRows);
+        for (uint32_t i = 0; i < nA; ++i) {
+            const uint32_t a_row0 = (uint32_t)rg.r0 + i * a_tile;
+            const uint32_t first = a_row0 / (uint32_t)kStripBRows + kPerTile;
+            if (first >= jend) {
+                dst.push_back({a_row0, 1, first, first, ks_data});
+                continue;
+            }
+            for (uint32_t j0 = first; j0 < jend; j0 += max_run)
+                dst.push_back({a_row0, (uint32_t)(j0 == first), j0,
+                               std::min(jend, j0 + max_run), ks_data});
+        }
+    }
+}
 static void build_strip_items(const StripShaping& sh, const std::vector<RowRange>& ranges,
                               uint32_t n_kslices, uint32_t shard_rank, uint32_t shard_count,
                               uint32_t a_tile, std::vector<StripItem>& items,
@@ -103,49 +138,34 @@
         if (pair_mode || strip_owns_slice(ks, shard_rank, shard_count)) slices_of[(local++ / xg) % 8].push_back(ks);
     std::vector<uint64_t> pair_load(shard_count, 0);
     auto emit_slice_all = [&](uint32_t ks, uint32_t max_run, std::vector<StripItem>& dst) {
-        const uint32_t ks_data = sh.one_slice_probe ? ks % 8u : ks;
-        for (const RowRange& rg : ranges) {
-            if (rg.back_from != ~0ull) {
-                const uint32_t blk0 = (uint32_t)(rg.r0 / kStripBRows);
-                for (uint64_t a0 = rg.back_from; a0 < rg.r1; a0 += a_tile) {
-                    const uint32_t a_row0 = (uint32_t)a0, end = (uint32_t)(a0 / kStripBRows);
-                    if (end <= blk0) {
-                        dst.push_back({a_row0, 1, end, end, ks_data});
-                        continue;
-                    }
-                    for (uint32_t j0 = blk0; j0 < end; j0 += max_run)
-                        dst.push_back({a_row0, (uint32_t)(j0 == blk0), j0, std::min(end, j0 + max_run), ks_data});
-                }
-                continue;
-            }
-            const uint64_t a_rows = (rg.a_end ? std::min(rg.a_end, rg.r1) : rg.r1) - rg.r0;
-            const uint32_t nA = (uint32_t)((a_rows + a_tile - 1) / a_tile);
-            const uint32_t jend = (uint32_t)((rg.r1 + kStripBRows - 1) / kStripBRows);
-            for (uint32_t i = 0; i < nA; ++i) {
-                const uint32_t a_row0 = (uint32_t)rg.r0 + i * a_tile;
-                const uint32_t first = a_row0 / (uint32_t)kStripBRows + kPerTile;
-                if (first >= jend) {
-                    dst.push_back({a_row0, 1, first, first, ks_data});
-                    continue;
-                }
-                for (uint32_t j0 = first; j0 < jend; j0 += max_run)
-                    dst.push_back({a_row0, (uint32_t)(j0 == first), j0,
-                                   std::min(jend, j0 + max_run), ks_data});
-            }
-        }
+        emit_strip_slice(ranges, a_tile, sh.one_slice_probe ? ks % 8u : ks, max_run, dst);
     };
     const uint32_t kTailLen = std::min(kMaxRun, kTailRun);
     std::vector<StripItem> proto_main, proto_tail;
     bool have_main = false, have_tail = false;
-    auto by_length = [&](const StripItem& p, const StripItem& q) {
-        return (p.j1 - p.j0) + p.diag * kPerTile > (q.j1 - q.j0) + q.diag * kPerTile;
+    uint32_t diag_mfmas[kStripRowsBlocks + 1] = {};
+    if (sh.rows_cost)
+        for (uint32_t nb = 0; nb <= kStripRowsBlocks; ++nb) diag_mfmas[nb] = strip_rows_item_mfmas(0, 1, 0, 0, nb * (uint32_t)kStripBRows);
+    auto length_of = [&](const StripItem& p) -> uint32_t {
+        if (!sh.rows_cost) return (p.j1 - p.j0) + p.diag * kPerTile;
+        return strip_rows_item_mfmas(p.a_row0, 0, p.j0, p.j1, sh.n_rows) + (p.diag ? diag_mfmas[strip_rows_real_blocks(p.a_row0, sh.n_rows)] : 0u);
+    };
+    auto by_length = [&](const StripItem& p, const StripItem& q) { return length_of(p) > length_of(q); };
+    auto longest_first = [&](std::vector<StripItem>& v) {
+        if (!sh.rows_cost) return std::stable_sort(v.begin(), v.end(), by_length);
+        std::vector<std::pair<uint32_t, uint32_t>> order(v.size());
+        for (size_t k = 0; k < v.size(); ++k) order[k] = {length_of(v[k]), (uint32_t)k};
+        std::stable_sort(order.begin(), order.end(), [](const auto& p, const auto& q) { return p.first > q.first; });
+        std::vector<StripItem> sorted(v.size());
+        for (size_t k = 0; k < v.size(); ++k) sorted[k] = v[order[k].second];
+        v.swap(sorted);
     };
     auto emit_copy = [&](uint32_t ks, uint32_t max_run, std::vector<StripItem>& dst) {
         std::vector<StripItem>& proto = max_run == kMaxRun ? proto_main : proto_tail;
         bool& have = max_run == kMaxRun ? have_main : have_tail;
         if (!have) {
             emit_slice_all(0u, max_run, proto);
-            if (max_run == kMaxRun) std::stable_sort(proto.begin(), proto.end(), by_length);
+            if (max_run == kMaxRun) longest_first(proto);
             have = true;
         }
         const uint32_t ks_data = sh.one_slice_probe ? ks % 8u : ks;
@@ -202,15 +222,10 @@
         std::vector<StripItem> tail;
         for (size_t k = n_main; k < sl.size(); ++k) emit_slice(sl[k], std::min(kMaxRun, kTailRun), tail);
         tail.insert(tail.end(), leftover_of[x].begin(), leftover_of[x].end());
-        std::stable_sort(tail.begin(), tail.end(), [&](const StripItem& p, const StripItem& q) {
-            return (p.j1 - p.j0) + p.diag * kPerTile > (q.j1 - q.j0) + q.diag * kPerTile;
-        });
+        longest_first(tail);
         per_xcd[x].insert(per_xcd[x].end(), tail.begin(), tail.end());
         if (per_xcd[x].size() <= (size_t)128 * (size_t)std::max(0, sh.lpt_rounds))
-            std::stable_sort(per_xcd[x].begin(), per_xcd[x].end(),
-                             [&](const StripItem& p, const StripItem& q) {
-                                 return (p.j1 - p.j0) + p.diag * kPerTile > (q.j1 - q.j0) + q.diag * kPerTile;
-                             });
+            longest_first(per_xcd[x]);
     }
     if (makespan) {
         auto cost_of = [&](const StripItem& it) { return (double)(it.j1 - it.j0) + (it.diag ? kPerTile + 3.0 : 0.0) + 5.0; };
@@ -247,6 +262,115 @@
     }
 }
 
+constexpr size_t kStripRowsWalkRounds = 4;
+static StripShaping choose_rows_tail(const StripShaping& now, const std::vector<RowRange>& ranges, uint32_t n_kslices, uint32_t a_tile,
+                                     uint32_t slots_per_xcd, bool run_is_set) {
+    const bool timing = timing_env();
+    uint32_t n_rows = kStripRowsNoTrim;
+    if (ranges.size() == 1 && ranges[0].r0 == 0 && ranges[0].a_end == 0 && ranges[0].back_from == ~0ull && ranges[0].r1 < (uint64_t)kStripRowsNoTrim)
+        n_rows = (uint32_t)ranges[0].r1;
+    uint32_t whole[8] = {}, left_over[8] = {}, local = 0;
+    const uint32_t modulo_slices = strip_modulo_slices(n_kslices, 1), xg = (uint32_t)std::max(1, now.xcd_group);
+    for (uint32_t ks = 0; ks < n_kslices; ++ks) ++(ks < modulo_slices ? whole : left_over)[(local++ / xg) % 8];
+    uint32_t x = 0;
+    for (uint32_t i = 1; i < 8; ++i)
+        if (whole[i] + left_over[i] > whole[x] + left_over[x]) x = i;
+    struct SliceCosts {
+        uint32_t run;
+        bool rows_cost;
+        std::vector<double> cost;
+        double sum;
+    };
+    std::vector<SliceCosts> slices;
+    slices.reserve(16);
+    auto slice_costs = [&](uint32_t run, bool rows_cost) -> const SliceCosts& {
+        for (const SliceCosts& sc : slices)
+            if (sc.run == run && sc.rows_cost == rows_cost) return sc;
+        std::vector<StripItem> items;
+        emit_strip_slice(ranges, a_tile, 0u, run, items);
+        std::vector<std::pair<uint32_t, uint32_t>> keyed(items.size());
+        for (size_t k = 0; k < items.size(); ++k) {
+            const StripItem& it = items[k];
+            const uint32_t mfmas = strip_rows_item_mfmas(it.a_row0, it.diag, it.j0, it.j1, n_rows);
+            keyed[k] = {rows_cost ? mfmas : (it.j1 - it.j0) + it.diag * (a_tile / (uint32_t)kStripBRows), mfmas};
+        }
+        std::stable_sort(keyed.begin(), keyed.end(), [](const auto& p, const auto& q) { return p.first > q.first; });
+        slices.push_back({run, rows_cost, {}, 0.0});
+        SliceCosts& sc = slices.back();
+        sc.cost.resize(keyed.size());
+        for (size_t k = 0; k < keyed.size(); ++k) sc.sum += sc.cost[k] = (double)keyed[k].second / kStripRowsStageMfmas;
+        return sc;
+    };
+    struct Walk {
+        std::vector<double> cost, resident;
+        double t0 = 0, makespan = 0;
+    };
+    std::vector<Walk> walks;
+    walks.reserve(8);
+    const uint32_t n_cus = std::max<uint32_t>(1, slots_per_xcd / 4u), n_slots = n_cus * 4u;
+    auto model = [&](const StripShaping& sh) {
+        const uint32_t run = (uint32_t)std::min(4096, std::max(1, sh.max_run));
+        const SliceCosts& main = slice_costs(run, sh.rows_cost);
+        const SliceCosts& tail = slice_costs(std::min(run, (uint32_t)std::min(4096, std::max(1, sh.tail_run))), sh.rows_cost);
+        const size_t n_main = whole[x] > (uint32_t)std::max(0, sh.tail_slices) ? whole[x] - (uint32_t)sh.tail_slices : 0;
+        const size_t n_tail = whole[x] - n_main + left_over[x];
+        const size_t in_main = n_main * main.cost.size(), n_list = in_main + n_tail * tail.cost.size();
+        walks.emplace_back();
+        Walk& w = walks.back();
+        if (n_list == 0) return 0.0;
+        auto at = [&](size_t k) { return k < in_main ? main.cost[k % main.cost.size()] : tail.cost[(k - in_main) / n_tail]; };
+        size_t start = n_list > kStripRowsWalkRounds * (size_t)n_slots ? n_list - kStripRowsWalkRounds * (size_t)n_slots : 0;
+        if (n_list <= (size_t)128 * (size_t)std::max(0, sh.lpt_rounds)) start = 0;
+        for (int pass = 0; pass < 2; ++pass) {
+            w.cost.resize(n_list - start);
+            double walked = 0;
+            for (size_t k = start; k < n_list; ++k) walked += w.cost[k - start] = at(k);
+            if (start == 0) break;
+            const double before = main.sum * (double)(n_main + n_tail) - walked;
+            double round = 0, held = 0;
+            for (uint32_t k = 0; k < n_slots; ++k) round += w.cost[k];
+            round /= (double)n_slots;
+            w.resident.resize(n_slots);
+            for (uint32_t c = 0; c < n_cus; ++c)
+                for (uint32_t s = 0; s < 4u; ++s) held += w.resident[c * 4u + s] = round * ((double)s + (double)(c + 1u) / (double)n_cus) / 4.0;
+            if (before >= 2.0 * held) {
+                w.t0 = (before - held) / (double)n_cus;
+                break;
+            }
+            w.resident.clear();
+            start = 0;
+        }
+        if (n_list <= (size_t)128 * (size_t)std::max(0, sh.lpt_rounds)) std::sort(w.cost.begin(), w.cost.end(), std::greater<double>());
+        for (size_t seen = 0; seen + 1 < walks.size(); ++seen)
+            if (walks[seen].t0 == w.t0 && walks[seen].cost == w.cost && walks[seen].resident == w.resident) return w.makespan = walks[seen].makespan;
+        return w.makespan = strip_rows_makespan(w.cost.data(), w.cost.size(), n_cus, 4u, kStripRowsStartStages, w.t0,
+                                                w.resident.empty() ? nullptr : w.resident.data());
+    };
+    StripShaping best = now;
+    double best_ms = model(now);
+    if (timing)
+        fprintf(stderr, "[strip plan] rows form, max_run %3d tail_run %2d tail_slices %2d (as it was): modelled makespan %.1f stages\n",
+                now.max_run, now.tail_run, now.tail_slices, best_ms);
+    for (const StripChoice& cand : kStripRowsShapings) {
+        if (run_is_set && cand.max_run != kStripRowsShapings[0].max_run) continue;
+        StripShaping trial = now;
+        trial.rows_cost = true;
+        trial.n_rows = n_rows;
+        if (!run_is_set) trial.max_run = cand.max_run;
+        trial.tail_run = cand.tail_run;
+        trial.tail_slices = cand.tail_slices;
+        const double ms = model(trial);
+        if (timing)
+            fprintf(stderr, "[strip plan] rows form, max_run %3d tail_run %2d tail_slices %2d: modelled makespan %.1f stages\n",
+                    trial.max_run, trial.tail_run, trial.tail_slices, ms);
+        if (ms < best_ms * 0.995) {
+            best = trial;
+            best_ms = ms;
+        }
+    }
+    return best;
+}
+
 static StripShaping choose_strip_shaping(const StripOptions& o, const std::vector<RowRange>& ranges, uint32_t n_kslices,
                                          uint32_t shard_count, uint32_t a_tile) {
     StripShaping sh;
@@ -258,9 +382,10 @@
     sh.one_slice_probe = o.one_slice_probe != 0;
     sh.pair_space = o.shard_pairs != 0;
     sh.max_run = o.max_run;
-    if (o.max_run != 0) return sh;
     const uint32_t slots = (uint32_t)std::max(1, o.n_cus / 8 * 4);
     const bool timing = timing_env();
+    const bool rows_tail = o.rows_form && o.tail_auto && shard_count == 1;
+    if (o.max_run != 0) return rows_tail ? choose_rows_tail(sh, ranges, n_kslices, a_tile, slots, true) : sh;
     double best = 0;
     for (int cand : {96, 64, 128}) {
         StripShaping trial = sh;
@@ -283,7 +408,7 @@
             best = worst;
         }
     }
-    return sh;
+    return rows_tail ? choose_rows_tail(sh, ranges, n_kslices, a_tile, slots, false) : sh;
 }
 
 StripRequest strip_request(const StripOptions& opt, const std::vector<RowRange>& ranges, uint32_t n_kslices,
@@ -299,9 +424,9 @@
 }
 
 void plan_strips(const StripRequest& rq, const std::vector<RowRange>& ranges, std::vector<StripItem>& items,
-                 uint32_t queue_base[8], uint32_t queue_count[8], int* run_chosen) {
+                 uint32_t queue_base[8], uint32_t queue_count[8], StripChoice* chosen) {
     const StripShaping sh = choose_strip_shaping(rq.opt, ranges, rq.n_kslices, rq.shard_count, rq.a_tile);
-    if (run_chosen) *run_chosen = sh.max_run;
+    if (chosen) *chosen = {sh.max_run, sh.tail_run, sh.tail_slices};
     build_strip_items(sh, ranges, rq.n_kslices, rq.shard_rank, rq.shard_count, rq.a_tile, items, queue_base, queue_count);
 }
 
@@ -1201,7 +1326,7 @@
                                      uint64_t capacity_items, uint64_t* n_items, int* run_chosen) {
     using namespace storm;
     if (!n_items || shard_count == 0 || shard_rank >= shard_count || n_words == 0 || form < 0 || form > 2 ||
-        max_run < 0 || max_run > 4096 || tail_run < 1 || tail_run > 4096 || tail_slices < 0 || tail_slices > 255 ||
+        max_run < 0 || max_run > 4096 || tail_run < 0 || tail_run > 4096 || tail_slices < 0 || tail_slices > 255 ||
         lpt_rounds < 0 || lpt_rounds > 63 || n_cus == 0) {
         set_error("strip_plan: bad arguments");
         return STORM_HIP_EINVAL;
@@ -1214,14 +1339,18 @@
         uint32_t qb[8], qc[8];
         StripOptions o;
         o.max_run = max_run;
-        o.tail_run = tail_run;
-        o.tail_slices = tail_slices;
+        o.tail_auto = tail_run == 0;
+        o.rows_form = form == 2;
+        o.tail_run = tail_run == 0 ? StripOptions().tail_run : tail_run;
+        o.tail_slices = tail_run == 0 ? StripOptions().tail_slices : tail_slices;
         o.lpt_rounds = lpt_rounds;
         o.shard_pairs = pair_space != 0;
         o.n_cus = (int)n_cus;
         o.xcd_group = form == 0 ? 1 : form == 1 ? 2 : (int)kStripRowsXcdGroup;
+        StripChoice used;
         plan_strips(strip_request(o, ranges, n_kslices, shard_rank, shard_count, form == 2 ? kStripRowsATile : (uint32_t)kStripATile),
-                    ranges, items, qb, qc, run_chosen);
+                    ranges, items, qb, qc, &used);
+        if (run_chosen) *run_chosen = tail_run == 0 ? used.max_run | used.tail_run << 16 | used.tail_slices << 24 : used.max_run;
         *n_items = items.size();
         if (out)
             for (uint64_t i = 0; i < std::min<uint64_t>(capacity_items, items.size()); ++i) {
@@ -1242,7 +1371,7 @@
                                      uint32_t shard_count, int form, int pair_space, uint32_t* out,
                                      uint64_t capacity_items, uint64_t* n_items) {
     const storm::StripOptions d;
-    return storm_hip_strip_plan3(n_rows, n_words, shard_rank, shard_count, form, pair_space, d.max_run, d.tail_run,
+    return storm_hip_strip_plan3(n_rows, n_words, shard_rank, shard_count, form, pair_space, d.max_run, 0 ,
                                  d.tail_slices, d.lpt_rounds, (uint32_t)d.n_cus, out, capacity_items, n_items, nullptr);
 }
 
diff --git a/stormbitmaps_amd/csrc/storm_hip_plan.h b/stormbitmaps_amd/csrc/storm_hip_plan.h
--- a/stormbitmaps_amd/csrc/storm_hip_plan.h
+++ b/stormbitmaps_amd/csrc/storm_hip_plan.h
@@ -1,5 +1,6 @@
 #pragma once
 
+#include <algorithm>
 #include <cstdint>
 #include <cstring>
 #include <type_traits>
@@ -89,6 +90,128 @@
 };
 static_assert(sizeof(StripItem) == 20, "read by device code");
 
+constexpr double kStripRowsStageMfmas = 128.0;
+inline double strip_rows_item_cost(const StripItem& it, uint32_t n_rows) {
+    return (double)strip_rows_item_mfmas(it.a_row0, it.diag, it.j0, it.j1, n_rows) / kStripRowsStageMfmas;
+}
+inline double strip_rows_makespan(const double* cost, size_t n_items, uint32_t n_cus, uint32_t slots_per_cu, double start_latency,
+                                  double t0 = 0.0, const double* resident = nullptr) {
+    if (n_cus == 0 || slots_per_cu == 0 || (n_items == 0 && !resident)) return t0;
+    constexpr double kNever = 1e300, kDone = 1e-9;
+    const size_t n_slots = (size_t)n_cus * slots_per_cu;
+    std::vector<double> left(n_slots, -1.0), ready(n_slots, t0), last(n_cus, t0), next(n_cus, kNever), tmp(slots_per_cu);
+    std::vector<uint32_t> held(n_cus, 0u);
+    auto step = [&](const double* r, double* l, double cur, double until, double* end) {
+        uint32_t working = 0;
+        double wake = kNever, least = kNever;
+        for (uint32_t s = 0; s < slots_per_cu; ++s) {
+            if (l[s] < 0.0) continue;
+            if (r[s] <= cur) {
+                ++working;
+                if (l[s] < least) least = l[s];
+            } else if (r[s] < wake)
+                wake = r[s];
+        }
+        *end = working ? cur + least * (double)working : kNever;
+        const double to = wake < until ? wake : until;
+        if (working && to > cur && to < kNever) {
+            const double each = (to - cur) / (double)working;
+            for (uint32_t s = 0; s < slots_per_cu; ++s)
+                if (l[s] >= 0.0 && r[s] <= cur) l[s] = l[s] > each ? l[s] - each : 0.0;
+        }
+        return to;
+    };
+    auto advance = [&](uint32_t c, double t) {
+        double end;
+        for (double cur = last[c]; cur < t;) cur = step(&ready[(size_t)c * slots_per_cu], &left[(size_t)c * slots_per_cu], cur, t, &end);
+        last[c] = t;
+    };
+    auto next_end = [&](uint32_t c) {
+        const double* r = &ready[(size_t)c * slots_per_cu];
+        for (uint32_t s = 0; s < slots_per_cu; ++s) tmp[s] = left[(size_t)c * slots_per_cu + s];
+        for (double cur = last[c];;) {
+            double end;
+            const double to = step(r, tmp.data(), cur, kNever, &end);
+            if (end <= to) return end;
+            cur = to;
+        }
+    };
+    uint32_t free_slots = (uint32_t)n_slots;
+    if (resident)
+        for (uint32_t c = 0; c < n_cus; ++c) {
+            for (uint32_t s = 0; s < slots_per_cu; ++s)
+                if (resident[(size_t)c * slots_per_cu + s] > kDone) {
+                    left[(size_t)c * slots_per_cu + s] = resident[(size_t)c * slots_per_cu + s];
+                    ++held[c];
+                    --free_slots;
+                }
+            next[c] = next_end(c);
+        }
+    size_t k = 0;
+    double now = t0;
+    constexpr uint32_t kNone = ~0u;
+    uint32_t only = kNone;
+    auto let_go = [&](uint32_t c) {
+        advance(c, now);
+        double* l = &left[(size_t)c * slots_per_cu];
+        uint32_t gone = 0;
+        for (uint32_t s = 0; s < slots_per_cu; ++s)
+            if (l[s] >= 0.0 && l[s] <= kDone && ready[(size_t)c * slots_per_cu + s] <= now) {
+                l[s] = -1.0;
+                ++gone;
+            }
+        held[c] -= gone;
+        free_slots += gone;
+        return gone;
+    };
+    for (;;) {
+        while (k < n_items && free_slots) {
+            uint32_t c = only != kNone ? only : 0u;
+            if (only == kNone)
+                for (uint32_t i = 1; i < n_cus; ++i)
+                    if (held[i] < held[c]) c = i;
+            advance(c, now);
+            double* l = &left[(size_t)c * slots_per_cu];
+            uint32_t s = 0;
+            while (l[s] >= 0.0) ++s;
+            l[s] = cost[k] > kDone ? cost[k] : 2.0 * kDone;
+            ++k;
+            ready[(size_t)c * slots_per_cu + s] = now + start_latency;
+            ++held[c];
+            --free_slots;
+            next[c] = next_end(c);
+        }
+        only = kNone;
+        uint32_t first = 0, ties = 1;
+        for (uint32_t i = 1; i < n_cus; ++i)
+            if (next[i] < next[first]) {
+                first = i;
+                ties = 1;
+            } else
+                ties += next[i] == next[first];
+        if (next[first] >= kNever) return now;
+        now = next[first];
+        if (ties == 1) {
+            if (let_go(first) && k < n_items)
+                only = first;
+            else
+                next[first] = next_end(first);
+            continue;
+        }
+        for (uint32_t c = first; c < n_cus; ++c)
+            if (next[c] <= now) {
+                let_go(c);
+                next[c] = next_end(c);
+            }
+    }
+}
+inline double strip_rows_makespan(const StripItem* list, size_t n_items, uint32_t n_rows, uint32_t n_cus, uint32_t slots_per_cu,
+                                  double start_latency) {
+    std::vector<double> cost(n_items);
+    for (size_t k = 0; k < n_items; ++k) cost[k] = strip_rows_item_cost(list[k], n_rows);
+    return strip_rows_makespan(cost.data(), n_items, n_cus, slots_per_cu, start_latency);
+}
+
 struct BitSeg {
     uint32_t a_blk;
     uint32_t ks;
@@ -147,7 +270,14 @@
     int32_t xcd_group = 1;
     int32_t persistent = 0;
     int32_t one_slice_probe = 0;
-};
+    int32_t rows_form = 0;
+    int32_t tail_auto = 0;
+};
+struct StripChoice {
+    int max_run = 0, tail_run = 0, tail_slices = 0;
+};
+constexpr StripChoice kStripRowsShapings[6] = {{96, 32, 12}, {96, 24, 8}, {64, 32, 12}, {64, 24, 8}, {128, 32, 12}, {128, 24, 8}};
+constexpr double kStripRowsStartStages = 8.0;
 struct StripRequest {
     StripOptions opt;
     uint32_t n_kslices, shard_rank, shard_count, a_tile;
@@ -158,7 +288,7 @@
 StripRequest strip_request(const StripOptions& opt, const std::vector<RowRange>& ranges, uint32_t n_kslices,
                            uint32_t shard_rank, uint32_t shard_count, uint32_t a_tile);
 void plan_strips(const StripRequest& rq, const std::vector<RowRange>& ranges, std::vector<StripItem>& items,
-                 uint32_t queue_base[8], uint32_t queue_count[8], int* run_chosen = nullptr);
+                 uint32_t queue_base[8], uint32_t queue_count[8], StripChoice* chosen = nullptr);
 
 void xcd_grouped_tiles(uint32_t i0, uint32_t i1, uint32_t j0, uint32_t j1, bool triangle,
                        std::vector<std::pair<uint16_t, uint16_t>>& out);
diff --git a/stormbitmaps_amd/dist.py b/stormbitmaps_amd/dist.py
--- a/stormbitmaps_amd/dist.py
+++ b/stormbitmaps_amd/dist.py
@@ -47,6 +47,8 @@
     if n.value:
         _lib.check(lib.storm_hip_strip_plan3(*args, out.ctypes.data_as(C.c_void_p), n.value, C.byref(n), C.byref(run)),
                    "storm_hip_strip_plan3")
+    if return_run and tail_run == 0:
+        return out, (run.value & 0xFFFF, run.value >> 16 & 0xFF, run.value >> 24 & 0xFF)
     return (out, int(run.value)) if return_run else out
 
 
```

Result: faster. 149200 billion words/s (median of 6 runs) (+1.4%).
